# baudm/parseq

Measured on NVIDIA H100. Metric: images/sec PARSeq-S 32x128 AR+1refine, higher is better.
Workload: dtype bf16

## Files before the change

### include/parseq_b200.h

```cpp
#ifndef PARSEQ_B200_H_
#define PARSEQ_B200_H_

#include <stdint.h>

#ifdef __cplusplus
extern "C" {
#endif

typedef struct parseq_engine parseq_engine;
typedef void* parseq_stream_t;

typedef enum parseq_status {
  PARSEQ_OK = 0,
  PARSEQ_ERR_INVALID_ARG = -1,
  PARSEQ_ERR_UNSUPPORTED = -2,
  PARSEQ_ERR_CUDA = -3,
  PARSEQ_ERR_STATE = -4,
  PARSEQ_ERR_NO_DEVICE = -5
} parseq_status;

typedef struct parseq_config {
  int32_t img_h, img_w;
  int32_t patch_h, patch_w;
  int32_t embed_dim;
  int32_t enc_num_heads, enc_mlp_ratio, enc_depth;
  int32_t dec_num_heads, dec_mlp_ratio, dec_depth;
  int32_t max_label_length;
  int32_t num_tokens;
  int32_t max_batch;
  int32_t device;
  int32_t arch;
} parseq_config;

int parseq_create(const parseq_config* cfg, parseq_engine** out);
void parseq_destroy(parseq_engine* e);

int parseq_set_weight(parseq_engine* e, const char* key, const float* data, int64_t numel);
int parseq_num_weights(const parseq_engine* e);
const char* parseq_weight_key(const parseq_engine* e, int i, int64_t* numel);

int parseq_finalize(parseq_engine* e, parseq_stream_t stream);

typedef struct parseq_forward_args {
  int32_t batch;
  int32_t max_length;
  int32_t decode_ar;
  int32_t refine_iters;
  const int32_t* forced_ids;
  const int32_t* forced_refine;
  const uint32_t* class_mask;
  float* attn_maps;
} parseq_forward_args;

int parseq_forward(parseq_engine* e, const parseq_forward_args* args, const float* images,
                   float* logits, int32_t* ids, int32_t* steps, parseq_stream_t stream);

int parseq_forward_host(parseq_engine* e, const parseq_forward_args* args, const float* images_host,
                        float* logits_host, int32_t* ids_host, int32_t* steps_host,
                        parseq_stream_t stream);

int parseq_forward_u8(parseq_engine* e, const parseq_forward_args* args, const uint8_t* images_hwc,
                      float* logits, int32_t* ids, int32_t* steps, parseq_stream_t stream);
int parseq_forward_host_u8(parseq_engine* e, const parseq_forward_args* args, const uint8_t* images_hwc_host,
                           float* logits_host, int32_t* ids_host, int32_t* steps_host, parseq_stream_t stream);
typedef struct parseq_crops {
  const uint8_t* data;
  int64_t data_bytes;
  const int64_t* offsets;
  const int32_t* sizes;
  int32_t rotation;
  const int32_t* rotations;
} parseq_crops;
int parseq_resize_crops(parseq_engine* e, int32_t batch, const parseq_crops* crops, uint8_t* out_hwc, parseq_stream_t stream);
int parseq_forward_crops(parseq_engine* e, const parseq_forward_args* args, const parseq_crops* crops, float* logits,
                         int32_t* ids, int32_t* steps, parseq_stream_t stream);
int parseq_forward_host_crops(parseq_engine* e, const parseq_forward_args* args, const parseq_crops* crops,
                              float* logits_host, int32_t* ids_host, int32_t* steps_host, parseq_stream_t stream);
typedef struct parseq_orient_args {
  int32_t num_orientations;
  int32_t orientations[4];
  float min_confidence;
  int32_t* rotation_out;
  float* confidence_out;
} parseq_orient_args;
int parseq_forward_crops_oriented(parseq_engine* e, const parseq_forward_args* args, const parseq_crops* crops,
                                  const parseq_orient_args* orient, float* logits, int32_t* ids, int32_t* steps,
                                  parseq_stream_t stream);
typedef struct parseq_score_args {
  int32_t batch;
  int32_t num_candidates;
  const int32_t* per_image;
  const int32_t* targets;
  const int32_t* lengths;
  float* attn_maps;
} parseq_score_args;
int parseq_score(parseq_engine* e, const parseq_score_args* a, const float* images, float* scores, float* token_logprobs,
                 parseq_stream_t stream);
int parseq_score_u8(parseq_engine* e, const parseq_score_args* a, const uint8_t* images_hwc, float* scores,
                    float* token_logprobs, parseq_stream_t stream);
int parseq_score_check(const parseq_config* cfg, const parseq_score_args* a);

typedef struct parseq_beam_args {
  int32_t batch, beam_width, max_length;
  const uint32_t* class_mask;
  float* attn_maps;
} parseq_beam_args;
int parseq_beam_search(parseq_engine* e, const parseq_beam_args* a, const float* images, int32_t* ids, int32_t* lengths,
                       float* scores, parseq_stream_t stream);
int parseq_beam_search_u8(parseq_engine* e, const parseq_beam_args* a, const uint8_t* images_hwc, int32_t* ids,
                          int32_t* lengths, float* scores, parseq_stream_t stream);

typedef struct parseq_lexicon parseq_lexicon;
typedef struct parseq_lexicon_desc {
  int32_t num_nodes, num_edges;
  const int32_t* first_edge;
  const int32_t* edge_class;
  const int32_t* edge_child;
  const uint8_t* terminal;
} parseq_lexicon_desc;
int parseq_lexicon_check(const parseq_config* cfg, const parseq_lexicon_desc* d);
int parseq_lexicon_create(parseq_engine* e, const parseq_lexicon_desc* d, parseq_lexicon** out, parseq_stream_t stream);
void parseq_lexicon_destroy(parseq_lexicon* lx);
int parseq_beam_search_lexicon(parseq_engine* e, const parseq_beam_args* a, const parseq_lexicon* lx, const int32_t* roots,
                               const float* images, int32_t* ids, int32_t* lengths, float* scores, parseq_stream_t stream);
int parseq_beam_search_lexicon_u8(parseq_engine* e, const parseq_beam_args* a, const parseq_lexicon* lx,
                                  const int32_t* roots, const uint8_t* images_hwc, int32_t* ids, int32_t* lengths,
                                  float* scores, parseq_stream_t stream);

int parseq_postprocess(const float* logits, int32_t batch, int32_t num_steps, int32_t num_classes, int32_t eos_id,
                       int32_t* ids, int32_t* lengths, float* confidence, parseq_stream_t stream);

int parseq_encode(parseq_engine* e, int32_t batch, const float* images, float* memory,
                  parseq_stream_t stream);

int parseq_decode(parseq_engine* e, int32_t batch, int32_t ctx_len, int32_t num_queries, const int32_t* tgt,
                  const float* memory, const float* query, const uint8_t* query_mask, const uint8_t* padding_mask,
                  float* out, parseq_stream_t stream);
int parseq_decode_ex(parseq_engine* e, int32_t batch, int32_t ctx_len, int32_t num_queries, const int32_t* tgt,
                     const float* memory, const float* query, const uint8_t* query_mask, const uint8_t* padding_mask,
                     const uint8_t* content_mask, float* out, parseq_stream_t stream);
int parseq_head(parseq_engine* e, int32_t rows, const float* x, float* logits, parseq_stream_t stream);
int parseq_text_embed(parseq_engine* e, int32_t n, const int32_t* ids, float* out, parseq_stream_t stream);

int64_t parseq_kernel_launches(const parseq_engine* e);
int parseq_bench_tma_stream(void* buf, int64_t bytes, int cluster, int ctas, int nboxes, int nslot, int mode, void* sink,
                            parseq_stream_t stream);
int64_t parseq_debug_int(parseq_engine* e, const char* name);
int parseq_set_option(parseq_engine* e, const char* name, int64_t value);
int parseq_get_timing(parseq_engine* e, int category, double* ms, double* flops, int64_t* count);
int parseq_get_ar_profile(parseq_engine* e, uint64_t* out512);
const char* parseq_last_error(void);
const char* parseq_version(void);

int parseq_gemm_bf16(const void* A, int64_t lda, const void* W, int64_t ldw, const float* bias,
                     int M, int N, int K, int mode, float alpha, const float* resid, int64_t ldr,
                     int resid_mod, void* out, int64_t ldo, parseq_stream_t stream);
int parseq_gemm_ln_bf16(const void* A, int64_t lda, const void* W, int64_t ldw, const float* bias,
                        int M, int D, int K, float* x_inout, const float* gamma, const float* beta,
                        float eps, void* xn_bf16, parseq_stream_t stream);
int parseq_mlp_ln_bf16(const void* xn, const void* W1, const float* b1, const void* W2, const float* b2,
                       int M, int D, float* x_inout, const float* gamma, const float* beta, float eps,
                       void* xn_out_bf16, parseq_stream_t stream);
int parseq_layernorm_bf16(const float* x, const float* gamma, const float* beta, float eps, int M,
                          int D, void* y_bf16, float* y_f32_or_null, parseq_stream_t stream);
int parseq_enc_attention(const void* qkv_bf16, int B, int T, int D, int heads, void* out_bf16,
                         parseq_stream_t stream);
int parseq_qkv_attention_bf16(const void* xn_bf16, const void* W_qkv, const float* b_qkv, int B, int T, int D,
                              int heads, void* out_bf16, parseq_stream_t stream);
int parseq_head_lse_bf16(const void* A, int64_t lda, const void* W, int64_t ldw, const float* bias, int M, int N, int K,
                         const int32_t* tgt, float* part, float* tlogit, parseq_stream_t stream);
int parseq_head_topk_bf16(const void* A, int64_t lda, const void* W, int64_t ldw, const float* bias, int M, int N, int K,
                          int k, const uint32_t* mask, int mask_div, float* part, uint64_t* keys, parseq_stream_t stream);
typedef struct parseq_beam_select_args {
  const float* logits;
  const float* part;
  const uint64_t* keys;
  int32_t ntiles;
  int64_t row0, img_stride, slot_stride;
  int32_t batch, num_classes, beam_width, step, num_steps;
  const uint32_t* class_mask;
  int32_t mask_ld;
  const int32_t* ids_in;
  const float* score_in;
  const int32_t* len_in;
  const int32_t* st_in;
  int32_t* ids_out;
  float* score_out;
  int32_t* len_out;
  int32_t* st_out;
  int32_t* parent;
  int32_t ids_ld;
  int32_t* out_ids;
  int32_t* out_len;
  float* out_score;
  const int32_t* first_edge;
  const int32_t* edge_class;
  const int32_t* edge_child;
  const uint8_t* terminal;
  const int32_t* roots;
  const int32_t* node_in;
  int32_t* node_out;
} parseq_beam_select_args;
int parseq_beam_select(const parseq_beam_select_args* a, parseq_stream_t stream);

#ifdef __cplusplus
}
#endif
#endif
```

### parseq_b200/csrc/engine.cu

```cuda
#include <cuda.h>
#include <cuda_runtime.h>

#include <algorithm>
#include <cmath>
#include <cstdio>
#include <cstdlib>
#include <cstring>
#include <functional>
#include <map>
#include <mutex>
#include <set>
#include <string>
#include <type_traits>
#include <vector>

#include "../../include/parseq_b200.h"
#include "gemm.cuh"
#include "kernels.cuh"
#include "dec_ar.cuh"
#include "dec_ar2.cuh"
#include "gemm_ln.cuh"
#include "mlp_ln.cuh"
#include "attn_wgmma.cuh"
#include "qkv_attn.cuh"
#include "crops.cuh"
#include "orient.cuh"
#include "owners.h"

namespace {

constexpr int kMaxHeadClasses = 16384;
constexpr int kMaxLabelLength = 63;

thread_local std::string g_last_error;

int fail(int code, const std::string& msg) {
  g_last_error = msg;
  return code;
}
#define PQ_CUDA(expr)                                                                              \
  do {                                                                                             \
    cudaError_t _e = (expr);                                                                       \
    if (_e != cudaSuccess)                                                                         \
      return fail(PARSEQ_ERR_CUDA, std::string(#expr) + " -> " + cudaGetErrorString(_e));          \
  } while (0)
#define PQ_TRY(expr)                 \
  do {                               \
    int _r = (expr);                 \
    if (_r != PARSEQ_OK) return _r;  \
  } while (0)

typedef CUresult (*PFN_encodeTiled)(CUtensorMap*, CUtensorMapDataType, cuuint32_t, void*, const cuuint64_t*,
                                    const cuuint64_t*, const cuuint32_t*, const cuuint32_t*, CUtensorMapInterleave,
                                    CUtensorMapSwizzle, CUtensorMapL2promotion, CUtensorMapFloatOOBfill);
PFN_encodeTiled g_encode = nullptr;

int load_driver_api() {
  if (g_encode != nullptr) return PARSEQ_OK;
  void* fn = nullptr;
  cudaDriverEntryPointQueryResult qres;
  cudaError_t e = cudaGetDriverEntryPoint("cuTensorMapEncodeTiled", &fn, cudaEnableDefault, &qres);
  if (e != cudaSuccess || fn == nullptr || qres != cudaDriverEntryPointSuccess)
    return fail(PARSEQ_ERR_CUDA, "cuTensorMapEncodeTiled not available from the driver");
  g_encode = reinterpret_cast<PFN_encodeTiled>(fn);
  return PARSEQ_OK;
}

int make_tmap(CUtensorMap* tm, const void* ptr, int esize, long long rows, long long cols, long long ld, int box_cols,
              int box_rows) {
  PQ_TRY(load_driver_api());
  if ((reinterpret_cast<uintptr_t>(ptr) & 15u) != 0 || ((ld * esize) & 15) != 0)
    return fail(PARSEQ_ERR_INVALID_ARG, "GEMM operand must be 16-byte aligned with a 16-byte multiple row stride");
  cuuint64_t dims[2] = {static_cast<cuuint64_t>(cols), static_cast<cuuint64_t>(rows)};
  cuuint64_t strides[1] = {static_cast<cuuint64_t>(ld) * static_cast<cuuint64_t>(esize)};
  cuuint32_t box[2] = {static_cast<cuuint32_t>(box_cols), static_cast<cuuint32_t>(box_rows)};
  cuuint32_t estr[2] = {1, 1};
  CUresult r = g_encode(tm, esize == 2 ? CU_TENSOR_MAP_DATA_TYPE_BFLOAT16 : CU_TENSOR_MAP_DATA_TYPE_FLOAT32, 2,
                        const_cast<void*>(ptr), dims, strides, box, estr,
                        CU_TENSOR_MAP_INTERLEAVE_NONE, CU_TENSOR_MAP_SWIZZLE_128B, CU_TENSOR_MAP_L2_PROMOTION_L2_256B,
                        CU_TENSOR_MAP_FLOAT_OOB_FILL_NONE);
  if (r != CUDA_SUCCESS) return fail(PARSEQ_ERR_CUDA, "cuTensorMapEncodeTiled failed: " + std::to_string(int(r)));
  return PARSEQ_OK;
}

int make_tmap3d(CUtensorMap* tm, const void* ptr, long long d0, long long d1, long long d2, long long ld1, long long ld2,
                int box_d0, int box_d1) {
  PQ_TRY(load_driver_api());
  if ((reinterpret_cast<uintptr_t>(ptr) & 15u) != 0 || ((ld1 * 2) & 15) != 0 || ((ld2 * 2) & 15) != 0)
    return fail(PARSEQ_ERR_INVALID_ARG, "tensor map operand must be 16-byte aligned with 16-byte multiple strides");
  cuuint64_t dims[3] = {static_cast<cuuint64_t>(d0), static_cast<cuuint64_t>(d1), static_cast<cuuint64_t>(d2)};
  cuuint64_t strides[2] = {static_cast<cuuint64_t>(ld1) * 2u, static_cast<cuuint64_t>(ld2) * 2u};
  cuuint32_t box[3] = {static_cast<cuuint32_t>(box_d0), static_cast<cuuint32_t>(box_d1), 1u};
  cuuint32_t estr[3] = {1, 1, 1};
  CUresult r = g_encode(tm, CU_TENSOR_MAP_DATA_TYPE_BFLOAT16, 3, const_cast<void*>(ptr), dims, strides, box, estr,
                        CU_TENSOR_MAP_INTERLEAVE_NONE, CU_TENSOR_MAP_SWIZZLE_128B, CU_TENSOR_MAP_L2_PROMOTION_L2_256B,
                        CU_TENSOR_MAP_FLOAT_OOB_FILL_NONE);
  if (r != CUDA_SUCCESS) return fail(PARSEQ_ERR_CUDA, "cuTensorMapEncodeTiled(3d) failed: " + std::to_string(int(r)));
  return PARSEQ_OK;
}

int make_tmap_kv4d(CUtensorMap* tm, const void* ptr, int T, int max_batch, int panels, int box_t) {
  PQ_TRY(load_driver_api());
  if ((reinterpret_cast<uintptr_t>(ptr) & 15u) != 0)
    return fail(PARSEQ_ERR_INVALID_ARG, "tensor map operand must be 16-byte aligned");
  const cuuint64_t row = 128;
  cuuint64_t dims[4] = {64, static_cast<cuuint64_t>(T), static_cast<cuuint64_t>(max_batch), static_cast<cuuint64_t>(panels)};
  cuuint64_t strides[3] = {row, row * T, row * T * max_batch};
  cuuint32_t box[4] = {64, static_cast<cuuint32_t>(box_t), 1u, 1u};
  cuuint32_t estr[4] = {1, 1, 1, 1};
  CUresult r = g_encode(tm, CU_TENSOR_MAP_DATA_TYPE_BFLOAT16, 4, const_cast<void*>(ptr), dims, strides, box, estr,
                        CU_TENSOR_MAP_INTERLEAVE_NONE, CU_TENSOR_MAP_SWIZZLE_128B, CU_TENSOR_MAP_L2_PROMOTION_L2_256B,
                        CU_TENSOR_MAP_FLOAT_OOB_FILL_NONE);
  if (r != CUDA_SUCCESS) return fail(PARSEQ_ERR_CUDA, "cuTensorMapEncodeTiled(K/V 4d) failed: " + std::to_string(int(r)));
  return PARSEQ_OK;
}

uint16_t f32_to_bf16_rne(float f) {
  uint32_t u;
  std::memcpy(&u, &f, 4);
  if ((u & 0x7fffffffu) > 0x7f800000u) return static_cast<uint16_t>((u >> 16) | 0x40u);
  u += 0x7fffu + ((u >> 16) & 1u);
  return static_cast<uint16_t>(u >> 16);
}

struct LaunchOpts {
  int sm_count = 0;
  bool use_pdl = true;
  int ln_cta_group = 0;
  int ln_split = 0;
  int mlp_cta_group = 0;
  bool pair_pdl = false;
  int gemm_stages = 0;
  int attn_impl = 0;
  int ln_clusters = 0;
};
LaunchOpts g_default_opts;

int ensure_sm_count(LaunchOpts& o) {
  if (o.sm_count == 0) {
    int dev = 0;
    PQ_CUDA(cudaGetDevice(&dev));
    PQ_CUDA(cudaDeviceGetAttribute(&o.sm_count, cudaDevAttrMultiProcessorCount, dev));
  }
  return PARSEQ_OK;
}

struct LaunchConfig {
  cudaLaunchConfig_t cfg{};
  cudaLaunchAttribute attr[2];
  LaunchConfig(dim3 grid, dim3 block, size_t smem, cudaStream_t st, unsigned cluster, bool pdl) {
    cfg.gridDim = grid;
    cfg.blockDim = block;
    cfg.dynamicSmemBytes = smem;
    cfg.stream = st;
    cfg.attrs = attr;
    if (cluster > 0) {
      attr[cfg.numAttrs].id = cudaLaunchAttributeClusterDimension;
      attr[cfg.numAttrs].val.clusterDim.x = cluster;
      attr[cfg.numAttrs].val.clusterDim.y = 1;
      attr[cfg.numAttrs].val.clusterDim.z = 1;
      ++cfg.numAttrs;
    }
    if (pdl) {
      attr[cfg.numAttrs].id = cudaLaunchAttributeProgrammaticStreamSerialization;
      attr[cfg.numAttrs].val.programmaticStreamSerializationAllowed = 1;
      ++cfg.numAttrs;
    }
  }
  LaunchConfig(const LaunchConfig&) = delete;
  LaunchConfig& operator=(const LaunchConfig&) = delete;
};

template <typename... KArgs, typename... Args>
int launch_ex(const LaunchConfig& lc, void (*kern)(KArgs...), const Args&... args) {
  PQ_CUDA(cudaLaunchKernelEx(&lc.cfg, kern, static_cast<KArgs>(args)...));
  return PARSEQ_OK;
}
template <typename... KArgs, typename... Args>
int launch_k(const LaunchOpts& lo, void (*kern)(KArgs...), dim3 grid, dim3 block, size_t smem, cudaStream_t st, const Args&... args) {
  return launch_ex(LaunchConfig(grid, block, smem, st, 0, lo.use_pdl), kern, args...);
}
bool cluster_pdl(const LaunchOpts& lo, int cg) { return lo.use_pdl && (cg == 1 || lo.pair_pdl); }

template <typename F>
int dispatch_width(int D, const char* what, F&& f) {
  switch (D) {
    case 192: return f(std::integral_constant<int, 192>{});
    case 384: return f(std::integral_constant<int, 384>{});
    case 768: return f(std::integral_constant<int, 768>{});
    default: return fail(PARSEQ_ERR_UNSUPPORTED, std::string(what) + ": embed_dim must be 192, 384 or 768");
  }
}

template <int EPI, int STORE>
int launch_gemm_cfg(const LaunchOpts& lo, const CUtensorMap& ta, const CUtensorMap& tb, const CUtensorMap& to,
                    const pq::GemmParams& p, int tiles, cudaStream_t st) {
  const int grid = tiles < lo.sm_count ? tiles : lo.sm_count;
  return launch_k(lo, pq::gemm_bf16_wgmma_kernel<EPI, STORE>, dim3(static_cast<unsigned>(grid)), dim3(pq::GEMM_THREADS),
                  pq::GemmCfg::smem_bytes<STORE != pq::ST_REG>(), st, ta, tb, to, p);
}

size_t head_smem_bytes(int C, int D) {
  return ((static_cast<size_t>(C) * (D / 2 + 1) * 4 + 15) / 16) * 16 + static_cast<size_t>(pq::HEAD_ROWS) * D * 4 +
         4 * pq::HEAD_ROWS * 128 * 4 + pq::HEAD_ROWS * 128 * 4;
}
int ln_head_argmax_launch(const LaunchOpts& lo, const float* y, const float* g, const float* b, float eps, const __nv_bfloat16* Wh, const float* bh,
                          int M, int C, int D, float* logits, long long logits_ld, int* ids, int ids_ld, int nq, int dst_off,
                          const int* forced, int forced_ld, const uint32_t* mask, cudaStream_t st) {
  if (C > 128) return fail(PARSEQ_ERR_UNSUPPORTED, "head kernel covers at most 128 classes");
  const dim3 grid((M + pq::HEAD_ROWS - 1) / pq::HEAD_ROWS), block(384);
  const size_t sm = head_smem_bytes(C, D);
  switch (D) {
    case 192: return launch_k(lo, pq::dec_ln_head_argmax_kernel<192>, grid, block, sm, st, y, g, b, eps, Wh, bh, M, C, logits,
                              logits_ld, ids, ids_ld, nq, dst_off, forced, forced_ld, mask);
    case 384: return launch_k(lo, pq::dec_ln_head_argmax_kernel<384>, grid, block, sm, st, y, g, b, eps, Wh, bh, M, C, logits,
                              logits_ld, ids, ids_ld, nq, dst_off, forced, forced_ld, mask);
    case 768: return launch_k(lo, pq::dec_ln_head_argmax_kernel<768>, grid, block, sm, st, y, g, b, eps, Wh, bh, M, C, logits,
                              logits_ld, ids, ids_ld, nq, dst_off, forced, forced_ld, mask);
    default: return fail(PARSEQ_ERR_UNSUPPORTED, "head kernel: embed_dim must be 192, 384 or 768");
  }
}

template <int D, int MT, int CS, bool HS, bool WIDE, int IDP>
constexpr auto ar2_kernel() {
  if constexpr (IDP == 64) {
    if constexpr (WIDE) return pq::dec_ar2_long_wide_kernel<D, MT, CS, HS>;
    else return pq::dec_ar2_long_kernel<D, MT, CS, HS>;
  } else {
    if constexpr (WIDE) return pq::dec_ar2_wide_kernel<D, MT, CS, HS>;
    else return pq::dec_ar2_kernel<D, MT, CS, HS>;
  }
}
template <typename... KArgs>
int set_smem(void (*kern)(KArgs...), size_t bytes) {
  PQ_CUDA(cudaFuncSetAttribute(kern, cudaFuncAttributeMaxDynamicSharedMemorySize, static_cast<int>(bytes)));
  return PARSEQ_OK;
}
template <int D, int MT, int CS, bool WIDE, int IDP>
int ar2_attr() {
  PQ_TRY(set_smem(ar2_kernel<D, MT, CS, false, WIDE, IDP>(), pq::dec_ar2_smem_bytes<D, MT, CS, IDP>()));
  if constexpr (MT == 1 && CS == 8 && D / 64 <= CS)
    PQ_TRY(set_smem(ar2_kernel<D, MT, CS, true, WIDE, IDP>(), pq::dec_ar2_smem_bytes<D, MT, CS, IDP>()));
  return PARSEQ_OK;
}
template <bool WIDE, int IDP>
int ar2_set_attributes() {
  PQ_TRY((ar2_attr<192, 1, 8, WIDE, IDP>())); PQ_TRY((ar2_attr<192, 2, 8, WIDE, IDP>())); PQ_TRY((ar2_attr<384, 1, 8, WIDE, IDP>()));
  PQ_TRY((ar2_attr<384, 2, 8, WIDE, IDP>())); PQ_TRY((ar2_attr<768, 1, 8, WIDE, IDP>()));
  PQ_TRY((ar2_attr<192, 1, 6, WIDE, IDP>())); PQ_TRY((ar2_attr<192, 2, 6, WIDE, IDP>())); PQ_TRY((ar2_attr<384, 1, 6, WIDE, IDP>()));
  PQ_TRY((ar2_attr<384, 2, 6, WIDE, IDP>())); PQ_TRY((ar2_attr<768, 1, 6, WIDE, IDP>()));
  return PARSEQ_OK;
}

template <int D, int MODE>
int gemm_ln_attr() { return set_smem(pq::gemm_ln_fused_kernel<D, MODE>, pq::GemmLnCfg<D, MODE>::kSmemBytes); }
template <int D, int CG>
int mlp_ln_attr() { return set_smem(pq::mlp_ln_fused_kernel<D, CG>, pq::MlpLnCfg<D, CG>::kSmemBytes); }
template <int NK>
int attn_wgmma_attr() { return set_smem(pq::enc_attention_wgmma_kernel<NK>, pq::atw_smem_bytes<NK>()); }
template <int D>
int qkv_attn_attr() { return set_smem(pq::enc_qkv_attn_kernel<D>, pq::QkvAttnCfg::kSmemBytes); }
template <int EPI, int STORE>
int gemm_attr() { return set_smem(pq::gemm_bf16_wgmma_kernel<EPI, STORE>, pq::GemmCfg::smem_bytes<STORE != pq::ST_REG>()); }
constexpr int kTmaBenchSmem = 12 * pq::A2_SLOT + 1024 + 256;

int init_kernel_attributes() {
  PQ_TRY(set_smem(pq::dec_ar_kernel<192, 1>, pq::dec_ar_smem_bytes<192>()));
  PQ_TRY(set_smem(pq::dec_ar_kernel<192, 2>, pq::dec_ar_smem_bytes<192>()));
  PQ_TRY(set_smem(pq::dec_ar_kernel<384, 1>, pq::dec_ar_smem_bytes<384>()));
  PQ_TRY(set_smem(pq::dec_ar_kernel<384, 2>, pq::dec_ar_smem_bytes<384>()));
  PQ_TRY(set_smem(pq::dec_ar_kernel<768, 1>, pq::dec_ar_smem_bytes<768>()));
  PQ_TRY(set_smem(pq::dec_ar_kernel<768, 2>, pq::dec_ar_smem_bytes<768>()));
  PQ_TRY((ar2_set_attributes<false, 32>()));
  PQ_TRY((ar2_set_attributes<true, 32>()));
  PQ_TRY((ar2_set_attributes<false, 64>()));
  PQ_TRY((ar2_set_attributes<true, 64>()));
  PQ_TRY(set_smem(pq::dec_ln_head_argmax_kernel<192>, 120 * 1024));
  PQ_TRY(set_smem(pq::dec_ln_head_argmax_kernel<384>, 160 * 1024));
  PQ_TRY(set_smem(pq::dec_ln_head_argmax_kernel<768>, 226 * 1024));
  PQ_TRY((gemm_ln_attr<192, 0>())); PQ_TRY((gemm_ln_attr<384, 0>())); PQ_TRY((gemm_ln_attr<192, 1>()));
  PQ_TRY((gemm_ln_attr<384, 1>())); PQ_TRY((gemm_ln_attr<384, 2>()));
  PQ_TRY((mlp_ln_attr<192, 1>())); PQ_TRY((mlp_ln_attr<384, 1>())); PQ_TRY((mlp_ln_attr<192, 2>())); PQ_TRY((mlp_ln_attr<384, 2>()));
  PQ_TRY((attn_wgmma_attr<128>())); PQ_TRY((attn_wgmma_attr<256>()));
  PQ_TRY((qkv_attn_attr<192>())); PQ_TRY((qkv_attn_attr<384>()));
  PQ_TRY((gemm_attr<pq::EPI_F32, pq::ST_REG>()));
  PQ_TRY((gemm_attr<pq::EPI_F32_RESID, pq::ST_REG>()));
  PQ_TRY((gemm_attr<pq::EPI_BF16, pq::ST_REG>()));
  PQ_TRY((gemm_attr<pq::EPI_BF16, pq::ST_TMA_2D>()));
  PQ_TRY((gemm_attr<pq::EPI_BF16, pq::ST_TMA_3D>()));
  PQ_TRY((gemm_attr<pq::EPI_GELU_BF16, pq::ST_REG>()));
  PQ_TRY((gemm_attr<pq::EPI_GELU_BF16, pq::ST_TMA_2D>()));
  PQ_TRY(set_smem(pq::gemm_bf16_lse_kernel, pq::GemmCfg::smem_bytes<false>()));
  PQ_TRY(set_smem(pq::gemm_bf16_topk_kernel, pq::GemmCfg::smem_bytes<false>()));
  PQ_TRY(set_smem(pq::tma_stream_bench_kernel, kTmaBenchSmem));
  int dev = 0, optin = 0;
  PQ_CUDA(cudaGetDevice(&dev));
  PQ_CUDA(cudaDeviceGetAttribute(&optin, cudaDevAttrMaxSharedMemoryPerBlockOptin, dev));
  PQ_TRY(set_smem(pq::crop_resize_bicubic_kernel, static_cast<size_t>(optin)));
  return PARSEQ_OK;
}

int ensure_kernel_attributes() {
  static std::mutex mu;
  static std::set<int> done;
  int dev = 0;
  PQ_CUDA(cudaGetDevice(&dev));
  std::lock_guard<std::mutex> lock(mu);
  if (done.count(dev) != 0) return PARSEQ_OK;
  PQ_TRY(init_kernel_attributes());
  done.insert(dev);
  return PARSEQ_OK;
}

int gemm_launch(LaunchOpts& lo, const void* A, long long lda, const void* W, long long ldw, const float* bias, int M, int N,
                int K, int mode, float alpha, const float* resid, long long ldr, int resid_mod, void* out, long long ldo,
                cudaStream_t st, long long blocked_rows = 0) {
  if (M <= 0 || N <= 0 || K <= 0) return fail(PARSEQ_ERR_INVALID_ARG, "gemm: empty problem");
  if (mode != pq::EPI_F32 && mode != pq::EPI_BF16 && mode != pq::EPI_GELU_BF16)
    return fail(PARSEQ_ERR_INVALID_ARG, "gemm: mode must be 0 (fp32), 1 (bf16) or 2 (GELU bf16)");
  PQ_TRY(ensure_sm_count(lo));
  CUtensorMap ta, tb, to;
  PQ_TRY(make_tmap(&ta, A, 2, M, K, lda, pq::GEMM_BLOCK_K, pq::GEMM_BLOCK_M));
  PQ_TRY(make_tmap(&tb, W, 2, N, K, ldw, pq::GEMM_BLOCK_K, pq::GEMM_BLOCK_N));
  pq::GemmParams p;
  p.M = M; p.N = N; p.K = K; p.alpha = alpha; p.bias = bias;
  p.resid = resid; p.ldr = ldr; p.resid_mod = resid_mod; p.out = out; p.ldo = ldo;
  const int esz = (mode == pq::EPI_F32) ? 4 : 2;
  bool vec = ((reinterpret_cast<uintptr_t>(out) & 7u) == 0) && ((ldo * esz) % 8 == 0);
  if (resid != nullptr) vec = vec && ((reinterpret_cast<uintptr_t>(resid) & 7u) == 0) && ((ldr * 4) % 8 == 0);
  p.vec_ok = vec ? 1 : 0;
  int store = pq::ST_REG;
  if (blocked_rows > 0) {
    if (mode != pq::EPI_BF16 || N % 64 != 0 || blocked_rows < M || (reinterpret_cast<uintptr_t>(out) & 15u) != 0)
      return fail(PARSEQ_ERR_INVALID_ARG, "gemm: blocked output needs a bf16 epilogue, N % 64 == 0 and rows >= M");
    PQ_TRY(make_tmap3d(&to, out, 64, M, N / 64, 64, 64 * blocked_rows, 64, pq::GEMM_BLOCK_M));
    store = pq::ST_TMA_3D;
  } else if (mode != pq::EPI_F32 && (reinterpret_cast<uintptr_t>(out) & 15u) == 0 && (ldo * 2) % 16 == 0 && ldo >= N) {
    PQ_TRY(make_tmap(&to, out, 2, M, N, ldo, 64, pq::GEMM_BLOCK_M));
    store = pq::ST_TMA_2D;
  } else {
    to = ta;
  }
  p.max_stages = lo.gemm_stages;
  p.num_m_tiles = (M + pq::GEMM_BLOCK_M - 1) / pq::GEMM_BLOCK_M;
  p.num_n_tiles = (N + pq::GEMM_BLOCK_N - 1) / pq::GEMM_BLOCK_N;
  const int tiles = p.num_m_tiles * p.num_n_tiles;
  if (mode == pq::EPI_F32)
    return resid != nullptr ? launch_gemm_cfg<pq::EPI_F32_RESID, pq::ST_REG>(lo, ta, tb, to, p, tiles, st)
                            : launch_gemm_cfg<pq::EPI_F32, pq::ST_REG>(lo, ta, tb, to, p, tiles, st);
  if (mode == pq::EPI_BF16) {
    if (store == pq::ST_TMA_3D) return launch_gemm_cfg<pq::EPI_BF16, pq::ST_TMA_3D>(lo, ta, tb, to, p, tiles, st);
    return store == pq::ST_TMA_2D ? launch_gemm_cfg<pq::EPI_BF16, pq::ST_TMA_2D>(lo, ta, tb, to, p, tiles, st)
                                  : launch_gemm_cfg<pq::EPI_BF16, pq::ST_REG>(lo, ta, tb, to, p, tiles, st);
  }
  return store == pq::ST_TMA_2D ? launch_gemm_cfg<pq::EPI_GELU_BF16, pq::ST_TMA_2D>(lo, ta, tb, to, p, tiles, st)
                                : launch_gemm_cfg<pq::EPI_GELU_BF16, pq::ST_REG>(lo, ta, tb, to, p, tiles, st);
}

int gemm_lse_launch(LaunchOpts& lo, const void* A, long long lda, const void* W, long long ldw, const float* bias, int M, int N,
                    int K, const int* tgt, float2* part, float* tlogit, cudaStream_t st) {
  if (M <= 0 || N <= 0 || K <= 0) return fail(PARSEQ_ERR_INVALID_ARG, "gemm: empty problem");
  PQ_TRY(ensure_sm_count(lo));
  CUtensorMap ta, tb;
  PQ_TRY(make_tmap(&ta, A, 2, M, K, lda, pq::GEMM_BLOCK_K, pq::GEMM_BLOCK_M));
  PQ_TRY(make_tmap(&tb, W, 2, N, K, ldw, pq::GEMM_BLOCK_K, pq::GEMM_BLOCK_N));
  pq::GemmParams p{};
  p.M = M; p.N = N; p.K = K; p.alpha = 1.0f; p.bias = bias;
  p.out = part;
  p.max_stages = lo.gemm_stages;
  p.num_m_tiles = (M + pq::GEMM_BLOCK_M - 1) / pq::GEMM_BLOCK_M;
  p.num_n_tiles = (N + pq::GEMM_BLOCK_N - 1) / pq::GEMM_BLOCK_N;
  p.lse_tgt = tgt;
  p.lse_tlogit = tlogit;
  const int tiles = p.num_m_tiles * p.num_n_tiles;
  return launch_k(lo, pq::gemm_bf16_lse_kernel, dim3(static_cast<unsigned>(tiles < lo.sm_count ? tiles : lo.sm_count)),
                  dim3(pq::GEMM_THREADS), pq::GemmCfg::smem_bytes<false>(), st, ta, tb, ta, p);
}

int gemm_topk_launch(LaunchOpts& lo, const void* A, long long lda, const void* W, long long ldw, const float* bias, int M, int N,
                     int K, int k, const uint32_t* mask, int mask_div, float2* part, unsigned long long* keys, cudaStream_t st) {
  if (M <= 0 || N <= 0 || K <= 0) return fail(PARSEQ_ERR_INVALID_ARG, "gemm: empty problem");
  PQ_TRY(ensure_sm_count(lo));
  CUtensorMap ta, tb;
  PQ_TRY(make_tmap(&ta, A, 2, M, K, lda, pq::GEMM_BLOCK_K, pq::GEMM_BLOCK_M));
  PQ_TRY(make_tmap(&tb, W, 2, N, K, ldw, pq::GEMM_BLOCK_K, pq::GEMM_BLOCK_N));
  pq::GemmParams p{};
  p.M = M; p.N = N; p.K = K; p.alpha = 1.0f; p.bias = bias;
  p.out = part;
  p.max_stages = lo.gemm_stages;
  p.num_m_tiles = (M + pq::GEMM_BLOCK_M - 1) / pq::GEMM_BLOCK_M;
  p.num_n_tiles = (N + pq::GEMM_BLOCK_N - 1) / pq::GEMM_BLOCK_N;
  p.topk_keys = keys;
  p.topk_k = k;
  p.topk_mask = mask;
  p.topk_mask_div = mask_div;
  const int tiles = p.num_m_tiles * p.num_n_tiles;
  return launch_k(lo, pq::gemm_bf16_topk_kernel, dim3(static_cast<unsigned>(tiles < lo.sm_count ? tiles : lo.sm_count)),
                  dim3(pq::GEMM_THREADS), pq::GemmCfg::smem_bytes<false>(), st, ta, tb, ta, p);
}

bool gemm_ln_supported(int D) { return D == 192 || D == 384; }
template <int D, int MODE>
int launch_gemm_ln(LaunchOpts& lo, const void* A, long long lda, const void* W, long long ldw, const float* bias, int M, int K, float* x,
                   const float* gamma, const float* beta, float eps, void* xn, cudaStream_t st) {
  using Cfg = pq::GemmLnCfg<D, MODE>;
  CUtensorMap ta, tb, tx;
  PQ_TRY(make_tmap(&ta, A, 2, M, K, lda, pq::GEMM_BLOCK_K, Cfg::kABox));
  PQ_TRY(make_tmap(&tb, W, 2, D, K, ldw, pq::GEMM_BLOCK_K, Cfg::kBox));
  if ((reinterpret_cast<uintptr_t>(x) & 7u) != 0 || (reinterpret_cast<uintptr_t>(xn) & 3u) != 0)
    return fail(PARSEQ_ERR_INVALID_ARG, "gemm_ln: x must be 8-byte and xn 4-byte aligned");
  pq::GemmLnParams p;
  p.M = M; p.K = K; p.bias = bias; p.gamma = gamma; p.beta = beta; p.eps = eps;
  p.num_m_tiles = (M + Cfg::kTileM - 1) / Cfg::kTileM;
  int clusters = p.num_m_tiles;
  if constexpr (MODE == 2) {
    PQ_TRY(make_tmap(&tx, x, 4, M, D, D, Cfg::kXBoxCols, pq::GLN_BLOCK_M));
    if (lo.ln_clusters == 0) {
      const LaunchConfig occ(dim3(static_cast<unsigned>(lo.sm_count / Cfg::kCG * Cfg::kCG)), dim3(pq::GLN_THREADS),
                             Cfg::kSmemBytes, st, Cfg::kCG, false);
      PQ_CUDA(cudaOccupancyMaxActiveClusters(&lo.ln_clusters, pq::gemm_ln_fused_kernel<D, MODE>, &occ.cfg));
      if (lo.ln_clusters <= 0) return fail(PARSEQ_ERR_CUDA, "gemm_ln: no cluster of the persistent kernel fits the device");
    }
    clusters = std::min(p.num_m_tiles, lo.ln_clusters);
  } else {
    tx = ta;
  }
  return launch_ex(LaunchConfig(dim3(static_cast<unsigned>(clusters * Cfg::kCG)), dim3(pq::GLN_THREADS), Cfg::kSmemBytes, st,
                                Cfg::kCG, cluster_pdl(lo, Cfg::kCG)),
                   pq::gemm_ln_fused_kernel<D, MODE>, ta, tb, tx, x, reinterpret_cast<__nv_bfloat16*>(xn), p);
}
int gemm_ln_launch(LaunchOpts& lo, const void* A, long long lda, const void* W, long long ldw, const float* bias, int M, int D,
                   int K, float* x, const float* gamma, const float* beta, float eps, void* xn, cudaStream_t st) {
  if (M <= 0 || K <= 0) return fail(PARSEQ_ERR_INVALID_ARG, "gemm_ln: empty problem");
  PQ_TRY(ensure_sm_count(lo));
  PQ_TRY(load_driver_api());
  if (D == 384 && lo.ln_split != 1)
    return launch_gemm_ln<384, 2>(lo, A, lda, W, ldw, bias, M, K, x, gamma, beta, eps, xn, st);
  if (lo.ln_cta_group == 2) {
    if (D == 384) return launch_gemm_ln<384, 1>(lo, A, lda, W, ldw, bias, M, K, x, gamma, beta, eps, xn, st);
    if (D == 192) return launch_gemm_ln<192, 1>(lo, A, lda, W, ldw, bias, M, K, x, gamma, beta, eps, xn, st);
  }
  if (D == 384) return launch_gemm_ln<384, 0>(lo, A, lda, W, ldw, bias, M, K, x, gamma, beta, eps, xn, st);
  if (D == 192) return launch_gemm_ln<192, 0>(lo, A, lda, W, ldw, bias, M, K, x, gamma, beta, eps, xn, st);
  return fail(PARSEQ_ERR_UNSUPPORTED, "gemm_ln: embed_dim must be 192 or 384");
}

template <int D, int CG>
int launch_mlp_ln(const LaunchOpts& lo, const void* xn, const void* W1, const float* b1, const void* W2, const float* b2, int M,
                  float* x, const float* gamma, const float* beta, float eps, void* xn_out, cudaStream_t st) {
  using Cfg = pq::MlpLnCfg<D, CG>;
  if ((reinterpret_cast<uintptr_t>(x) & 7u) != 0 || (reinterpret_cast<uintptr_t>(xn_out) & 3u) != 0)
    return fail(PARSEQ_ERR_INVALID_ARG, "mlp_ln: x must be 8-byte and xn_out 4-byte aligned");
  CUtensorMap txn, tw1, tw2;
  PQ_TRY(make_tmap(&txn, xn, 2, M, D, D, 64, pq::GLN_BLOCK_M));
  PQ_TRY(make_tmap(&tw1, W1, 2, Cfg::kH, D, D, 64, Cfg::kW1Rows));
  PQ_TRY(make_tmap(&tw2, W2, 2, D, Cfg::kH, Cfg::kH, 64, Cfg::kW2Rows));
  pq::MlpLnParams p;
  p.M = M; p.b1 = b1; p.b2 = b2; p.gamma = gamma; p.beta = beta; p.eps = eps;
  p.num_m_tiles = (M + pq::GLN_BLOCK_M * CG - 1) / (pq::GLN_BLOCK_M * CG);
  return launch_ex(LaunchConfig(dim3(static_cast<unsigned>(p.num_m_tiles * CG)), dim3(pq::MLP_THREADS), Cfg::kSmemBytes, st, CG,
                                cluster_pdl(lo, CG)),
                   pq::mlp_ln_fused_kernel<D, CG>, txn, tw1, tw2, x, reinterpret_cast<__nv_bfloat16*>(xn_out), p);
}
int mlp_ln_launch(LaunchOpts& lo, const void* xn, const void* W1, const float* b1, const void* W2, const float* b2, int M, int D,
                  float* x, const float* gamma, const float* beta, float eps, void* xn_out, cudaStream_t st) {
  if (M <= 0) return fail(PARSEQ_ERR_INVALID_ARG, "mlp_ln: empty problem");
  PQ_TRY(ensure_sm_count(lo));
  PQ_TRY(load_driver_api());
  const int CG = lo.mlp_cta_group ? lo.mlp_cta_group : 2;
  if (CG == 2) {
    if (D == 384) return launch_mlp_ln<384, 2>(lo, xn, W1, b1, W2, b2, M, x, gamma, beta, eps, xn_out, st);
    if (D == 192) return launch_mlp_ln<192, 2>(lo, xn, W1, b1, W2, b2, M, x, gamma, beta, eps, xn_out, st);
  }
  if (D == 384) return launch_mlp_ln<384, 1>(lo, xn, W1, b1, W2, b2, M, x, gamma, beta, eps, xn_out, st);
  if (D == 192) return launch_mlp_ln<192, 1>(lo, xn, W1, b1, W2, b2, M, x, gamma, beta, eps, xn_out, st);
  return fail(PARSEQ_ERR_UNSUPPORTED, "mlp_ln: embed_dim must be 192 or 384 (hidden width 4 * embed_dim)");
}

int layernorm_launch(const LaunchOpts& lo, const float* x, const float* g, const float* b, float eps, int M, int D, void* y, float* y32,
                     cudaStream_t st, const float* add = nullptr, int add_mod = 1, float* xw = nullptr) {
  const int rows_per_block = 8;
  const int grid = (M + rows_per_block - 1) / rows_per_block;
  __nv_bfloat16* yb = reinterpret_cast<__nv_bfloat16*>(y);
  switch (D) {
    case 192: return launch_k(lo, pq::layernorm_kernel<192>, dim3(grid), dim3(256), 0, st, x, g, b, eps, M, yb, y32, add, add_mod, xw);
    case 384: return launch_k(lo, pq::layernorm_kernel<384>, dim3(grid), dim3(256), 0, st, x, g, b, eps, M, yb, y32, add, add_mod, xw);
    case 768: return launch_k(lo, pq::layernorm_kernel<768>, dim3(grid), dim3(256), 0, st, x, g, b, eps, M, yb, y32, add, add_mod, xw);
    default: return fail(PARSEQ_ERR_UNSUPPORTED, "layernorm: embed_dim must be 192, 384 or 768");
  }
}

int enc_attention_launch(const LaunchOpts& lo, const void* qkv, int B, int T, int D, int heads, void* out, cudaStream_t st) {
  if (D != heads * pq::ATT_DH) return fail(PARSEQ_ERR_UNSUPPORTED, "encoder attention kernels cover head_dim=64");
  if (lo.attn_impl == 1 && T <= 256) {
    const dim3 grid(static_cast<unsigned>(B * heads), static_cast<unsigned>((T + 127) / 128));
    const __nv_bfloat16* q = reinterpret_cast<const __nv_bfloat16*>(qkv);
    __nv_bfloat16* o = reinterpret_cast<__nv_bfloat16*>(out);
    if (T <= 128)
      return launch_k(lo, pq::enc_attention_wgmma_kernel<128>, grid, dim3(pq::ATW_THREADS), pq::atw_smem_bytes<128>(), st, q, o, T, D, heads);
    return launch_k(lo, pq::enc_attention_wgmma_kernel<256>, grid, dim3(pq::ATW_THREADS), pq::atw_smem_bytes<256>(), st, q, o, T, D, heads);
  }
  if (T != pq::ATT_T) {
    return launch_k(lo, pq::enc_attention_any_kernel, dim3(B * heads, (T + pq::ATT_T - 1) / pq::ATT_T), dim3(256), 0, st,
                    reinterpret_cast<const __nv_bfloat16*>(qkv), reinterpret_cast<__nv_bfloat16*>(out), T, D, heads);
  }
  return launch_k(lo, pq::enc_attention_kernel, dim3(B * heads), dim3(256), 0, st,
                  reinterpret_cast<const __nv_bfloat16*>(qkv), reinterpret_cast<__nv_bfloat16*>(out), D, heads);
}

bool qkv_attn_supported(int T, int D, int heads) { return T == pq::ATT_T && D == heads * pq::ATT_DH && (D == 192 || D == 384); }
int qkv_attn_launch(LaunchOpts& lo, const void* xn, const void* W, const float* bias, int B, int T, int D, int heads, void* out,
                    cudaStream_t st) {
  if (B <= 0) return fail(PARSEQ_ERR_INVALID_ARG, "qkv_attn: empty batch");
  if (!qkv_attn_supported(T, D, heads))
    return fail(PARSEQ_ERR_UNSUPPORTED, "qkv_attn: T = 128, head_dim 64 and embed_dim 192 or 384 only");
  if ((reinterpret_cast<uintptr_t>(out) & 15u) != 0) return fail(PARSEQ_ERR_INVALID_ARG, "qkv_attn: out must be 16-byte aligned");
  PQ_TRY(ensure_sm_count(lo));
  CUtensorMap tx, tw;
  PQ_TRY(make_tmap(&tx, xn, 2, static_cast<long long>(B) * T, D, D, pq::GEMM_BLOCK_K, pq::ATT_T));
  PQ_TRY(make_tmap(&tw, W, 2, 3 * D, D, D, pq::GEMM_BLOCK_K, pq::ATT_DH));
  const int items = B * heads;
  const dim3 grid(static_cast<unsigned>(items < lo.sm_count ? items : lo.sm_count));
  __nv_bfloat16* o = reinterpret_cast<__nv_bfloat16*>(out);
  if (D == 192)
    return launch_k(lo, pq::enc_qkv_attn_kernel<192>, grid, dim3(pq::QA_THREADS), pq::QkvAttnCfg::kSmemBytes, st, tx, tw, bias, o, items);
  return launch_k(lo, pq::enc_qkv_attn_kernel<384>, grid, dim3(pq::QA_THREADS), pq::QkvAttnCfg::kSmemBytes, st, tx, tw, bias, o, items);
}

int make_stream(Stream* s) {
  cudaStream_t h = nullptr;
  PQ_CUDA(cudaStreamCreateWithFlags(&h, cudaStreamNonBlocking));
  *s = Stream(h);
  return PARSEQ_OK;
}
int make_event(Event* ev) {
  cudaEvent_t h = nullptr;
  PQ_CUDA(cudaEventCreateWithFlags(&h, cudaEventDisableTiming));
  *ev = Event(h);
  return PARSEQ_OK;
}

struct Slot {
  std::string key;
  std::string pub;
  long long numel;
  bool bf16;
  DevBuf<unsigned char> dev;
  bool set;
};

struct Workspace {
  DevBuf<__nv_bfloat16> a_pe, xn, qkv, att, hid;
  DevBuf<float> x;
  DevBuf<float> vt_rows;
  DevBuf<__nv_bfloat16> mem, ckv;
  std::vector<DevBuf<__nv_bfloat16>> ckv_deep;
  DevBuf<__nv_bfloat16> ar_sa, ar_ca, ar_hd;
  DevBuf<float> ar_y, ar_qc, ar_part;
  DevBuf<int> ar_ids;
  DevBuf<unsigned int> ar_bar;
  DevBuf<unsigned long long> ar_prof;
  Event ev_enc;
  struct Stage {
    DevBuf<__nv_bfloat16> sa, yn, ca, hd;
    DevBuf<float> y, qc;
    DevBuf<int> ids_ar, ids_ctx;
    DevBuf<float> cx;
    std::vector<DevBuf<__nv_bfloat16>> kvc;
    DevBuf<float2> lse_part;
    DevBuf<float> lse_tlogit;
    struct Beam {
      int rows = 0;
      DevBuf<int> ids[2];
      DevBuf<float> score[2];
      DevBuf<int> len[2];
      DevBuf<int> st[2];
      DevBuf<int> parent;
      DevBuf<float> logits;
      DevBuf<float2> part;
      DevBuf<unsigned long long> keys;
      std::vector<DevBuf<__nv_bfloat16>> kvc;
      DevBuf<int> node[2];
    } bm;
    Stream stream;
    Event ev_done;
  };
  std::vector<Stage> stages;
  DevBuf<float> in_images, out_logits;
  DevBuf<int> out_ids, out_steps;
  DevBuf<float> out_maps;
  DevBuf<uint8_t> in_images_u8;
  DevBuf<uint32_t> in_mask;
  DevBuf<pq::CropDesc> crop_tab;
  DevBuf<int> sc_meta;
  DevBuf<unsigned char> sc_causal;
  DevBuf<float2> sc_vt_part;
  long long beam_bytes = 0;
  DevBuf<int> lex_roots;
  DevBuf<int> or_rd, or_steps;
  DevBuf<float> or_conf;
};

}

struct parseq_engine : Workspace {
  parseq_config cfg;
  int D, T, Kp, Me, Md, L, V, C, gh, gw, dh_dec;
  int ids_ld = 32;
  int arch = 0, Tp = 0;
  std::map<std::string, int> pub_index;
  int chunk;
  std::vector<Slot> slots;
  std::map<std::string, int> index;
  bool finalized = false;
  bool broken = false;
  LaunchOpts lo;
  long long launches = 0;
  bool timing = false;
  struct TimedLaunch { int cat; double flops; Event a, b; };
  std::vector<TimedLaunch> timed;
  std::vector<Event> event_pool;
  int cur_cat = 5;
  DevBuf<__nv_bfloat16> kvtab;
  DevBuf<float> qs;
  int dec_chunk = 128;
  int ar_kernel = 2;
  pq::DecAr2Maps ar2_maps[2];
  bool ar2_maps_ok = false;
  int ar2_clusters[3][2] = {{0, 0}, {0, 0}, {0, 0}};
  int ar2_occ[3][2] = {{0, 0}, {0, 0}, {0, 0}};
  int ar_last_cs = 0;
  int ar_last_per = 0, ar_last_ncl = 0;
  int ar_last_mt = 0, ar_last_hs = 0, ar_last_wide = 0, ar_last_idp = 0;
  int ar_last_path = -1;
  int ar_cs = 0;
  int ar_clusters_override = 0;
  int fuse_mlp = 0;
  int fuse_ln = 3;
  bool ar_prof_on = false;
  int max_batch = 512;
  Stream main;
  Stream copy;
  Event ev_c[3];
  Event ev_in, ev_out;
  int mask_ld = 0;
  std::vector<pq::CropDesc> crop_descs;
  long long crop_base = 0;
  DevBuf<uint8_t> crop_stage;
  bool use_graph = true;
  long long orient_rereads = 0, orient_readings = 0;
  struct GraphEntry { GraphExec exec; long long kernels; };
  std::map<std::vector<int>, GraphEntry> graphs;

  void* w(const std::string& k) const { return slots[index.at(k)].dev; }
  const float* wf(const std::string& k) const { return reinterpret_cast<const float*>(w(k)); }
  const __nv_bfloat16* wb(const std::string& k) const { return reinterpret_cast<const __nv_bfloat16*>(w(k)); }
};

struct parseq_lexicon {
  int device = 0, C = 0, V = 0, E = 0;
  DevBuf<int> first_edge;
  DevBuf<int> edge_class;
  DevBuf<int> edge_child;
  DevBuf<unsigned char> terminal;
};

template <typename T>
int DevBuf<T>::alloc(long long n) {
  reset();
  void* p = nullptr;
  PQ_CUDA(cudaMalloc(&p, static_cast<size_t>(n) * sizeof(T)));
  p_ = static_cast<T*>(p);
  n_ = n;
  g_live_bytes += bytes();
  return PARSEQ_OK;
}

template <typename T>
int DevBuf<T>::grow(const parseq_engine* e, long long n) {
  if (n <= n_) return PARSEQ_OK;
  if (p_ != nullptr) {
    PQ_CUDA(cudaStreamSynchronize(e->main));
    PQ_CUDA(cudaStreamSynchronize(e->copy));
  }
  return alloc(n);
}

namespace {

void add_slot(parseq_engine* e, const std::string& key, long long numel, bool bf16) {
  std::string pub = key;
  if (e->arch == 1 && key.rfind("encoder.", 0) == 0) pub = key.substr(8);
  e->index[key] = static_cast<int>(e->slots.size());
  e->pub_index[pub] = static_cast<int>(e->slots.size());
  e->slots.push_back(Slot{key, pub, numel, bf16, {}, false});
}

int check_ready(const parseq_engine* e, bool weights = true) {
  if (e == nullptr) return fail(PARSEQ_ERR_INVALID_ARG, "null argument");
  if (e->broken) return fail(PARSEQ_ERR_STATE, "engine workspace is gone (a failed resize): destroy the handle");
  if (weights && !e->finalized)
    return fail(PARSEQ_ERR_STATE, "parseq_finalize has not been called after the last weight update");
  return PARSEQ_OK;
}

int enter_main(parseq_engine* e, cudaStream_t user) {
  PQ_CUDA(cudaEventRecord(e->ev_in, user));
  PQ_CUDA(cudaStreamWaitEvent(e->main, e->ev_in, 0));
  return PARSEQ_OK;
}
int leave_main(parseq_engine* e, cudaStream_t user) {
  PQ_CUDA(cudaEventRecord(e->ev_out, e->main));
  PQ_CUDA(cudaStreamWaitEvent(user, e->ev_out, 0));
  return PARSEQ_OK;
}

long long image_bytes(const parseq_engine* e, bool u8) { return 3ll * e->cfg.img_h * e->cfg.img_w * (u8 ? 1 : 4); }

int alloc_workspace(parseq_engine* e) {
  const long long R = static_cast<long long>(e->chunk) * e->T;
  const long long RB = static_cast<long long>(e->max_batch) * e->T;
  const long long Rd = static_cast<long long>(e->dec_chunk) * e->L;
  const int D = e->D;
  PQ_TRY(e->a_pe.alloc(R * e->Kp));
  PQ_TRY(e->x.alloc(R * D));
  PQ_TRY(e->xn.alloc(R * D));
  PQ_TRY(e->qkv.alloc(R * 3 * D));
  PQ_TRY(e->att.alloc(R * D));
  PQ_TRY(e->hid.alloc(R * e->Me));
  PQ_TRY(e->mem.alloc(RB * D));
  PQ_TRY(e->ckv.alloc(RB * 2 * D));
  if (e->cfg.dec_depth > 1) {
    e->ckv_deep.resize(static_cast<size_t>(e->cfg.dec_depth - 1));
    for (auto& c : e->ckv_deep) PQ_TRY(c.alloc(RB * 2 * D));
  }
  PQ_TRY(e->ar_sa.alloc(1ll * e->max_batch * D));
  PQ_TRY(e->ar_ca.alloc(1ll * e->max_batch * D));
  PQ_TRY(e->ar_hd.alloc(1ll * e->max_batch * e->Md));
  PQ_TRY(e->ar_y.alloc(1ll * e->max_batch * D));
  PQ_TRY(e->ar_qc.alloc(1ll * e->max_batch * D));
// ... 2002 lines not shown
  return beam_lexicon_call(e, a, lx, roots, images, false, ids, lengths, scores, stream);
}

int parseq_beam_search_lexicon_u8(parseq_engine* e, const parseq_beam_args* a, const parseq_lexicon* lx,
                                  const int32_t* roots, const uint8_t* images_hwc, int32_t* ids, int32_t* lengths,
                                  float* scores, parseq_stream_t stream) {
  return beam_lexicon_call(e, a, lx, roots, images_hwc, true, ids, lengths, scores, stream);
}

int parseq_postprocess(const float* logits, int32_t batch, int32_t num_steps, int32_t num_classes, int32_t eos_id, int32_t* ids,
                       int32_t* lengths, float* confidence, parseq_stream_t stream) {
  if (logits == nullptr || ids == nullptr || lengths == nullptr || confidence == nullptr)
    return fail(PARSEQ_ERR_INVALID_ARG, "null argument");
  if (batch <= 0) return batch == 0 ? PARSEQ_OK : fail(PARSEQ_ERR_INVALID_ARG, "negative batch");
  pq::postprocess_kernel<<<(batch + 7) / 8, 256, 0, reinterpret_cast<cudaStream_t>(stream)>>>(logits, batch, num_steps, num_classes,
                                                                                              eos_id, ids, lengths, confidence);
  PQ_CUDA(cudaGetLastError());
  return PARSEQ_OK;
}

int parseq_encode(parseq_engine* e, int32_t batch, const float* images, float* memory, parseq_stream_t stream) {
  if (images == nullptr || memory == nullptr) return fail(PARSEQ_ERR_INVALID_ARG, "null argument");
  PQ_TRY(check_ready(e));
  PQ_CUDA(cudaSetDevice(e->cfg.device));
  cudaStream_t user = reinterpret_cast<cudaStream_t>(stream);
  PQ_TRY(enter_main(e, user));
  const long long img_sz = 3ll * e->cfg.img_h * e->cfg.img_w;
  for (int b0 = 0; b0 < batch; b0 += e->chunk) {
    const int B = (batch - b0 < e->chunk) ? (batch - b0) : e->chunk;
    PQ_TRY(encode_chunk(e, images + b0 * img_sz, false, B, e->mem, memory + 1ll * b0 * e->T * e->D, e->main));
  }
  return leave_main(e, user);
}

int parseq_decode(parseq_engine* e, int32_t batch, int32_t ctx_len, int32_t num_queries, const int32_t* tgt, const float* memory,
                  const float* query, const uint8_t* query_mask, const uint8_t* padding_mask, float* out,
                  parseq_stream_t stream) {
  return parseq_decode_ex(e, batch, ctx_len, num_queries, tgt, memory, query, query_mask, padding_mask, nullptr, out, stream);
}

int parseq_decode_ex(parseq_engine* e, int32_t batch, int32_t ctx_len, int32_t num_queries, const int32_t* tgt,
                     const float* memory, const float* query, const uint8_t* query_mask, const uint8_t* padding_mask,
                     const uint8_t* content_mask, float* out, parseq_stream_t stream) {
  if (tgt == nullptr || memory == nullptr || out == nullptr) return fail(PARSEQ_ERR_INVALID_ARG, "null argument");
  PQ_TRY(check_ready(e));
  if (e->arch != 0) return fail(PARSEQ_ERR_UNSUPPORTED, "decode: PARSeq only");
  if (batch < 0 || ctx_len < 1 || ctx_len > e->L || num_queries < 1 || num_queries > e->L)
    return fail(PARSEQ_ERR_INVALID_ARG, "decode: 1 <= context length, queries <= max_label_length + 1");
  if (batch == 0) return PARSEQ_OK;
  PQ_CUDA(cudaSetDevice(e->cfg.device));
  cudaStream_t user = reinterpret_cast<cudaStream_t>(stream);
  PQ_TRY(enter_main(e, user));
  const int D = e->D, T = e->T, J = ctx_len, NQ = num_queries;
  parseq_engine::Stage& sg = e->stages[0];
  cudaStream_t st = e->main;
  for (int b0 = 0; b0 < batch; b0 += e->dec_chunk) {
    const int Bc = (batch - b0 < e->dec_chunk) ? (batch - b0) : e->dec_chunk;
    const long long n4 = 1ll * Bc * T * D / 4;
    pq::f32_to_bf16_kernel<<<static_cast<unsigned>(std::min<long long>((n4 + 255) / 256, 132ll * 8)), 256, 0, st>>>(
        reinterpret_cast<const float4*>(memory + 1ll * b0 * T * D), reinterpret_cast<uint2*>(e->mem.get()), n4);
    PQ_CUDA(cudaGetLastError());
    PQ_TRY(cross_kv(e, Bc));
    pq::copy_ids_kernel<<<(Bc * e->ids_ld + 255) / 256, 256, 0, st>>>(tgt + 1ll * b0 * J, J, sg.ids_ctx, Bc, e->ids_ld);
    PQ_CUDA(cudaGetLastError());
    e->launches += 2;
    DecodeExtras ex;
    ex.query = query ? query + 1ll * b0 * NQ * D : nullptr;
    ex.qmask = query_mask;
    ex.pmask = padding_mask ? padding_mask + 1ll * b0 * J : nullptr;
    ex.cmask = content_mask;
    ex.out_norm = out + 1ll * b0 * NQ * D;
    PQ_TRY(decode_pass(e, sg, 0, Bc, NQ, 0, J, 0, sg.ids_ctx, nullptr, 0, nullptr, 0, nullptr, 0, nullptr, st, &ex));
  }
  return leave_main(e, user);
}

int parseq_head(parseq_engine* e, int32_t rows, const float* x, float* logits, parseq_stream_t stream) {
  if (x == nullptr || logits == nullptr) return fail(PARSEQ_ERR_INVALID_ARG, "null argument");
  PQ_TRY(check_ready(e));
  if (rows <= 0) return rows == 0 ? PARSEQ_OK : fail(PARSEQ_ERR_INVALID_ARG, "negative rows");
  PQ_CUDA(cudaSetDevice(e->cfg.device));
  cudaStream_t user = reinterpret_cast<cudaStream_t>(stream);
  PQ_TRY(enter_main(e, user));
  const int D = e->D;
  const int cap = e->dec_chunk * e->L;
  parseq_engine::Stage& sg = e->stages[0];
  for (int r0 = 0; r0 < rows; r0 += cap) {
    const int n = (rows - r0 < cap) ? (rows - r0) : cap;
    const long long n4 = 1ll * n * D / 4;
    pq::f32_to_bf16_kernel<<<static_cast<unsigned>(std::min<long long>((n4 + 255) / 256, 132ll * 8)), 256, 0, e->main>>>(
        reinterpret_cast<const float4*>(x + 1ll * r0 * D), reinterpret_cast<uint2*>(sg.yn.get()), n4);
    PQ_CUDA(cudaGetLastError());
    e->launches++;
    e->cur_cat = CAT_DEC_GEMM;
    PQ_TRY(gemm(e, sg.yn, D, e->w("head.weight"), D, e->wf("head.bias"), n, e->C, D, pq::EPI_F32, 1.0f, nullptr, 0, 0,
                logits + 1ll * r0 * e->C, e->C, e->main));
  }
  return leave_main(e, user);
}

int parseq_text_embed(parseq_engine* e, int32_t n, const int32_t* ids, float* out, parseq_stream_t stream) {
  if (e == nullptr || ids == nullptr || out == nullptr) return fail(PARSEQ_ERR_INVALID_ARG, "null argument");
  if (e->arch != 0) return fail(PARSEQ_ERR_UNSUPPORTED, "text_embed: PARSeq only");
  if (n <= 0) return n == 0 ? PARSEQ_OK : fail(PARSEQ_ERR_INVALID_ARG, "negative count");
  if (!e->slots[e->index.at("text_embed.embedding.weight")].set) return fail(PARSEQ_ERR_STATE, "weights not set");
  PQ_CUDA(cudaSetDevice(e->cfg.device));
  const long long total = 1ll * n * e->D;
  pq::text_embed_kernel<<<static_cast<unsigned>(std::min<long long>((total + 255) / 256, 132ll * 8)), 256, 0,
                          reinterpret_cast<cudaStream_t>(stream)>>>(ids, e->wf("text_embed.embedding.weight"), out, n, e->D, e->V,
                                                                    std::sqrt(static_cast<float>(e->D)));
  PQ_CUDA(cudaGetLastError());
  return PARSEQ_OK;
}

int parseq_bench_tma_stream(void* buf, int64_t bytes, int cluster, int ctas, int nboxes, int nslot, int mode, void* sink,
                            parseq_stream_t stream) {
  if (buf == nullptr || sink == nullptr || cluster < 1 || cluster > 8 || ctas % cluster != 0 || nslot < 1 || nslot > 12)
    return fail(PARSEQ_ERR_INVALID_ARG, "bench_tma_stream: bad arguments");
  const long long rows_total = 8192;
  const int blocks = static_cast<int>(bytes / (rows_total * 128));
  if (blocks < 1) return fail(PARSEQ_ERR_INVALID_ARG, "bench_tma_stream: buffer too small");
  PQ_TRY(ensure_kernel_attributes());
  CUtensorMap map;
  PQ_TRY(make_tmap3d(&map, buf, 64, rows_total, blocks, 64, 64 * rows_total, 64, 128));
  return launch_ex(LaunchConfig(dim3(static_cast<unsigned>(ctas)), dim3(pq::A2_THREADS + 32), kTmaBenchSmem,
                                reinterpret_cast<cudaStream_t>(stream), cluster > 1 ? static_cast<unsigned>(cluster) : 0, false),
                   pq::tma_stream_bench_kernel, map, nboxes, nslot, static_cast<int>(rows_total / 128), blocks, mode,
                   static_cast<unsigned int*>(sink));
}

int64_t parseq_debug_int(parseq_engine* e, const char* name) {
  if (name == nullptr) return -1;
  const std::string n(name);
  if (n == "ln_clusters") return (e ? e->lo : g_default_opts).ln_clusters;
  if (n == "live_device_bytes") return g_live_bytes;
  if (n == "live_cuda_objects") return g_live_objects;
  if (e == nullptr) return -1;
  if (n == "ar2_occupancy_mt1_cs8") return e->ar2_occ[1][0];
  if (n == "ar2_occupancy_mt2_cs8") return e->ar2_occ[2][0];
  if (n == "ar2_occupancy_mt1_cs6") return e->ar2_occ[1][1];
  if (n == "ar2_occupancy_mt2_cs6") return e->ar2_occ[2][1];
  if (n == "ar_last_cluster_size") return e->ar_last_cs;
  if (n == "ar_last_per") return e->ar_last_per;
  if (n == "ar_last_clusters") return e->ar_last_ncl;
  if (n == "ar_last_mt") return e->ar_last_mt;
  if (n == "ar_last_head_split") return e->ar_last_hs;
  if (n == "ar_last_wide") return e->ar_last_wide;
  if (n == "ar_last_ids_pitch") return e->ar_last_idp;
  if (n == "ar_last_path") return e->ar_last_path;
  if (n == "sm_count") return e->lo.sm_count;
  if (n == "beam_bytes") return e->beam_bytes;
  if (n == "orient_rereads") return e->orient_rereads;
  if (n == "orient_readings") return e->orient_readings;
  return -1;
}
int64_t parseq_kernel_launches(const parseq_engine* e) { return e ? e->launches : 0; }

int parseq_set_option(parseq_engine* e, const char* name, int64_t value) {
  if (name == nullptr) return fail(PARSEQ_ERR_INVALID_ARG, "null option");
  const std::string n(name);
  LaunchOpts& lo = e ? e->lo : g_default_opts;
  if (n == "block_n") {
    if (value != 0 && value != 64 && value != 128 && value != 192 && value != 256)
      return fail(PARSEQ_ERR_INVALID_ARG, "block_n: 0/64/128/192/256");
    return PARSEQ_OK;
  }
  if (n == "cta_group") {
    if (value < 0 || value > 2) return fail(PARSEQ_ERR_INVALID_ARG, "cta_group: 0 (auto) / 1 / 2");
    return PARSEQ_OK;
  }
  if (n == "attn_impl") { lo.attn_impl = value != 0 ? 1 : 0; if (e) e->graphs.clear(); return PARSEQ_OK; }
  if (n == "pdl") { lo.use_pdl = value != 0; if (e) e->graphs.clear(); return PARSEQ_OK; }
  if (n == "gemm_stages") {
    if (value < 0 || value == 1) return fail(PARSEQ_ERR_INVALID_ARG, "gemm_stages: 0 (full ring) or >= 2");
    lo.gemm_stages = static_cast<int>(value);
    if (e) e->graphs.clear();
    return PARSEQ_OK;
  }
  if (n == "ln_cta_group") {
    if (value < 0 || value > 2) return fail(PARSEQ_ERR_INVALID_ARG, "ln_cta_group: 0 (auto) / 1 / 2");
    lo.ln_cta_group = static_cast<int>(value);
    if (e) e->graphs.clear();
    return PARSEQ_OK;
  }
  if (n == "ln_split") {
    if (value < 0 || value > 2) return fail(PARSEQ_ERR_INVALID_ARG, "ln_split: 0 (auto) / 1 (off) / 2 (on)");
    lo.ln_split = static_cast<int>(value);
    if (e) e->graphs.clear();
    return PARSEQ_OK;
  }
  if (n == "mlp_cta_group") {
    if (value < 0 || value > 2) return fail(PARSEQ_ERR_INVALID_ARG, "mlp_cta_group: 0 (auto) / 1 / 2");
    lo.mlp_cta_group = static_cast<int>(value);
    if (e) e->graphs.clear();
    return PARSEQ_OK;
  }
  if (n == "pair_pdl") { lo.pair_pdl = value != 0; if (e) e->graphs.clear(); return PARSEQ_OK; }
  if (n == "fuse_mlp") {
    if (e == nullptr) return fail(PARSEQ_ERR_INVALID_ARG, "null engine");
    e->fuse_mlp = value != 0 ? 1 : 0;
    e->graphs.clear();
    return PARSEQ_OK;
  }
  if (n == "fuse_ln") {
    if (e == nullptr) return fail(PARSEQ_ERR_INVALID_ARG, "null engine");
    e->fuse_ln = static_cast<int>(value) & 7;
    e->graphs.clear();
    return PARSEQ_OK;
  }
  if (e == nullptr) return fail(PARSEQ_ERR_INVALID_ARG, "null engine");
  if (n == "timing") {
    e->timing = value != 0;
    for (auto& t : e->timed) { e->event_pool.push_back(std::move(t.a)); e->event_pool.push_back(std::move(t.b)); }
    e->timed.clear();
    return PARSEQ_OK;
  }
  if (n == "use_graph") { e->use_graph = value != 0; return PARSEQ_OK; }
  if (n == "ar_prof") { e->ar_prof_on = value != 0; e->graphs.clear(); return PARSEQ_OK; }
  if (n == "ar_clusters") {
    if (value < 0 || value > 1024) return fail(PARSEQ_ERR_INVALID_ARG, "ar_clusters out of range");
    e->ar_clusters_override = static_cast<int>(value);
    for (auto& r : e->ar2_clusters) r[0] = r[1] = 0;
    e->graphs.clear();
    return PARSEQ_OK;
  }
  if (n == "ar_cluster_size") {
    if (value != 0 && value != 6 && value != 8) return fail(PARSEQ_ERR_INVALID_ARG, "ar_cluster_size: 0 (auto) / 6 / 8");
    e->ar_cs = static_cast<int>(value);
    e->graphs.clear();
    return PARSEQ_OK;
  }
  if (n == "ar_kernel") {
    if (value < 0 || value > 2) return fail(PARSEQ_ERR_INVALID_ARG, "ar_kernel: 0 / 1 / 2");
    if (value == 1)
      if (const char* why = grid_barrier_limit(e)) return fail(PARSEQ_ERR_UNSUPPORTED, why);
    e->ar_kernel = static_cast<int>(value);
    e->graphs.clear();
    return PARSEQ_OK;
  }
  if (n == "chunk" || n == "max_batch" || n == "dec_chunk") {
    if (value <= 0 || value > 8192) return fail(PARSEQ_ERR_INVALID_ARG, "chunk / max_batch / dec_chunk out of range");
    int chunk = e->chunk, dec_chunk = e->dec_chunk, max_batch = e->max_batch;
    if (n == "chunk") chunk = static_cast<int>(value);
    else if (n == "dec_chunk") dec_chunk = static_cast<int>(value);
    else { max_batch = static_cast<int>(value); chunk = max_batch; }
    if (chunk > max_batch) chunk = max_batch;
    if (dec_chunk > max_batch) dec_chunk = max_batch;
    if ((max_batch + dec_chunk - 1) / dec_chunk > 64) return fail(PARSEQ_ERR_INVALID_ARG, "too many decoder chains");
    PQ_CUDA(cudaSetDevice(e->cfg.device));
    PQ_CUDA(cudaDeviceSynchronize());
    const int old_chunk = e->chunk, old_dec = e->dec_chunk, old_max = e->max_batch;
    free_workspace(e);
    e->chunk = chunk; e->dec_chunk = dec_chunk; e->max_batch = max_batch;
    int r = alloc_workspace(e);
    if (r != PARSEQ_OK) {
      const std::string why = g_last_error;
      free_workspace(e);
      e->chunk = old_chunk; e->dec_chunk = old_dec; e->max_batch = old_max;
      if (alloc_workspace(e) != PARSEQ_OK) { e->finalized = false; free_workspace(e); e->broken = true; }
      return fail(r, why);
    }
    return PARSEQ_OK;
  }
  return fail(PARSEQ_ERR_INVALID_ARG, "unknown option: " + n);
}

int parseq_get_ar_profile(parseq_engine* e, uint64_t* out512) {
  if (e == nullptr || out512 == nullptr) return fail(PARSEQ_ERR_INVALID_ARG, "null argument");
  PQ_CUDA(cudaMemcpy(out512, e->ar_prof, 32 * 16 * 8, cudaMemcpyDeviceToHost));
  return PARSEQ_OK;
}

int parseq_get_timing(parseq_engine* e, int category, double* ms, double* flops, int64_t* count) {
  if (e == nullptr || category < 0 || category >= CAT_COUNT) return fail(PARSEQ_ERR_INVALID_ARG, "bad timing query");
  double tms = 0.0, tf = 0.0;
  int64_t n = 0;
  for (auto& t : e->timed) {
    if (t.cat != category) continue;
    float dt = 0.f;
    cudaError_t ce = cudaEventElapsedTime(&dt, t.a, t.b);
    if (ce != cudaSuccess) return fail(PARSEQ_ERR_CUDA, std::string("timing readback: ") + cudaGetErrorString(ce));
    tms += dt; tf += t.flops; ++n;
  }
  if (ms) *ms = tms;
  if (flops) *flops = tf;
  if (count) *count = n;
  return PARSEQ_OK;
}

int parseq_gemm_bf16(const void* A, int64_t lda, const void* W, int64_t ldw, const float* bias, int M, int N, int K,
                     int mode, float alpha, const float* resid, int64_t ldr, int resid_mod, void* out, int64_t ldo,
                     parseq_stream_t stream) {
  if (mode < 0 || mode > 2) return fail(PARSEQ_ERR_INVALID_ARG, "bad epilogue mode");
  PQ_TRY(ensure_kernel_attributes());
  return gemm_launch(g_default_opts, A, lda, W, ldw, bias, M, N, K, mode, alpha, resid, ldr, resid_mod, out, ldo,
                     reinterpret_cast<cudaStream_t>(stream));
}
int parseq_gemm_ln_bf16(const void* A, int64_t lda, const void* W, int64_t ldw, const float* bias, int M, int D, int K,
                         float* x_inout, const float* gamma, const float* beta, float eps, void* xn_bf16,
                         parseq_stream_t stream) {
  PQ_TRY(ensure_kernel_attributes());
  return gemm_ln_launch(g_default_opts, A, lda, W, ldw, bias, M, D, K, x_inout, gamma, beta, eps, xn_bf16, reinterpret_cast<cudaStream_t>(stream));
}
int parseq_mlp_ln_bf16(const void* xn, const void* W1, const float* b1, const void* W2, const float* b2, int M, int D,
                       float* x_inout, const float* gamma, const float* beta, float eps, void* xn_out_bf16, parseq_stream_t stream) {
  PQ_TRY(ensure_kernel_attributes());
  return mlp_ln_launch(g_default_opts, xn, W1, b1, W2, b2, M, D, x_inout, gamma, beta, eps, xn_out_bf16,
                       reinterpret_cast<cudaStream_t>(stream));
}
int parseq_layernorm_bf16(const float* x, const float* gamma, const float* beta, float eps, int M, int D, void* y_bf16,
                          float* y_f32_or_null, parseq_stream_t stream) {
  PQ_TRY(ensure_kernel_attributes());
  return layernorm_launch(g_default_opts, x, gamma, beta, eps, M, D, y_bf16, y_f32_or_null, reinterpret_cast<cudaStream_t>(stream));
}
int parseq_enc_attention(const void* qkv_bf16, int B, int T, int D, int heads, void* out_bf16, parseq_stream_t stream) {
  PQ_TRY(ensure_kernel_attributes());
  PQ_TRY(ensure_sm_count(g_default_opts));
  return enc_attention_launch(g_default_opts, qkv_bf16, B, T, D, heads, out_bf16, reinterpret_cast<cudaStream_t>(stream));
}
int parseq_qkv_attention_bf16(const void* xn_bf16, const void* W_qkv, const float* b_qkv, int B, int T, int D, int heads,
                              void* out_bf16, parseq_stream_t stream) {
  PQ_TRY(ensure_kernel_attributes());
  return qkv_attn_launch(g_default_opts, xn_bf16, W_qkv, b_qkv, B, T, D, heads, out_bf16, reinterpret_cast<cudaStream_t>(stream));
}
int parseq_head_lse_bf16(const void* A, int64_t lda, const void* W, int64_t ldw, const float* bias, int M, int N, int K,
                         const int32_t* tgt, float* part, float* tlogit, parseq_stream_t stream) {
  if (part == nullptr || (tgt == nullptr) != (tlogit == nullptr))
    return fail(PARSEQ_ERR_INVALID_ARG, "head_lse: part is required, tgt and tlogit go together");
  PQ_TRY(ensure_kernel_attributes());
  return gemm_lse_launch(g_default_opts, A, lda, W, ldw, bias, M, N, K, tgt, reinterpret_cast<float2*>(part), tlogit,
                         reinterpret_cast<cudaStream_t>(stream));
}
int parseq_head_topk_bf16(const void* A, int64_t lda, const void* W, int64_t ldw, const float* bias, int M, int N, int K,
                          int k, const uint32_t* mask, int mask_div, float* part, uint64_t* keys, parseq_stream_t stream) {
  if (k < 1 || k > pq::BEAM_TOPK_LD) return fail(PARSEQ_ERR_INVALID_ARG, "head_topk: k must be in 1..16");
  if (part == nullptr || keys == nullptr) return fail(PARSEQ_ERR_INVALID_ARG, "head_topk: part and keys are required");
  if (mask != nullptr && mask_div < 1) return fail(PARSEQ_ERR_INVALID_ARG, "head_topk: mask_div must be >= 1");
  PQ_TRY(ensure_kernel_attributes());
  return gemm_topk_launch(g_default_opts, A, lda, W, ldw, bias, M, N, K, k, mask, mask != nullptr ? mask_div : 1,
                          reinterpret_cast<float2*>(part), reinterpret_cast<unsigned long long*>(keys),
                          reinterpret_cast<cudaStream_t>(stream));
}
int parseq_beam_select(const parseq_beam_select_args* a, parseq_stream_t stream) {
  if (a == nullptr) return fail(PARSEQ_ERR_INVALID_ARG, "beam_select: null arguments");
  const int C = a->num_classes, K = a->beam_width;
  const bool lex = a->first_edge != nullptr;
  if (a->batch < 1 || C < 1) return fail(PARSEQ_ERR_INVALID_ARG, "beam_select: batch and num_classes must be >= 1");
  if (K < 1 || K > pq::BEAM_MAX) return fail(PARSEQ_ERR_INVALID_ARG, "beam_select: beam_width must be in 1..16");
  if (a->ntiles != (C + pq::GEMM_BLOCK_N - 1) / pq::GEMM_BLOCK_N)
    return fail(PARSEQ_ERR_INVALID_ARG, "beam_select: ntiles must be ceil(num_classes / 128)");
  if (a->step < 0 || a->step >= a->num_steps) return fail(PARSEQ_ERR_INVALID_ARG, "beam_select: need 0 <= step < num_steps");
  if (a->ids_ld <= a->num_steps) return fail(PARSEQ_ERR_INVALID_ARG, "beam_select: ids_ld must exceed num_steps");
  if (a->logits == nullptr && (a->keys == nullptr || lex))
    return fail(PARSEQ_ERR_INVALID_ARG, "beam_select: logits are required without keys and with a lexicon");
  if (a->keys != nullptr && a->part == nullptr) return fail(PARSEQ_ERR_INVALID_ARG, "beam_select: keys need part");
  if (a->class_mask != nullptr && a->mask_ld < (C + 31) / 32)
    return fail(PARSEQ_ERR_INVALID_ARG, "beam_select: mask_ld must be >= ceil(num_classes / 32)");
  if (a->ids_in == nullptr || a->score_in == nullptr || a->len_in == nullptr || a->st_in == nullptr || a->ids_out == nullptr ||
      a->score_out == nullptr || a->len_out == nullptr || a->st_out == nullptr || a->parent == nullptr ||
      (a->step + 1 == a->num_steps && (a->out_ids == nullptr || a->out_len == nullptr || a->out_score == nullptr)))
    return fail(PARSEQ_ERR_INVALID_ARG, "beam_select: missing state or output array");
  if (lex && (a->edge_class == nullptr || a->edge_child == nullptr || a->terminal == nullptr || a->node_out == nullptr ||
              (a->step > 0 && a->node_in == nullptr)))
    return fail(PARSEQ_ERR_INVALID_ARG, "beam_select: incomplete lexicon");
  PQ_TRY(ensure_kernel_attributes());
  pq::BeamLex bl{};
  if (lex) bl = pq::BeamLex{a->first_edge, a->edge_class, a->edge_child, a->terminal, a->roots, a->node_in, a->node_out};
  return launch_k(g_default_opts, lex ? pq::beam_select_kernel<true> : pq::beam_select_kernel<false>,
                  dim3(static_cast<unsigned>(a->batch)), dim3(pq::BEAM_THREADS), 0, reinterpret_cast<cudaStream_t>(stream),
                  a->logits, reinterpret_cast<const float2*>(a->part),
                  reinterpret_cast<const unsigned long long*>(lex ? nullptr : a->keys), a->ntiles, static_cast<long long>(a->row0),
                  static_cast<long long>(a->img_stride), static_cast<long long>(a->slot_stride), C, K, a->step, a->num_steps,
                  a->class_mask, a->mask_ld, a->ids_in, a->score_in, a->len_in, a->st_in, a->ids_out, a->score_out, a->len_out,
                  a->st_out, a->parent, a->ids_ld, a->out_ids, a->out_len, a->out_score, bl);
}

}
```

### parseq_b200/csrc/gemm_ln.cuh

```cuda
#pragma once
#include "gemm.cuh"

namespace pq {

struct GemmLnParams {
  int M, K;
  const float* bias;
  const float* gamma;
  const float* beta;
  float eps;
  int num_m_tiles;
};

constexpr int GLN_THREADS = 384;
constexpr int GLN_BLOCK_M = 64;

template <int D, int MODE>
struct GemmLnCfg {
  static_assert(MODE == 0 || MODE == 1, "MODE");
  static constexpr int kCG = MODE == 0 ? 1 : 2;
  static constexpr int kTileM = GLN_BLOCK_M * kCG;
  static constexpr int kCols = D;
  static constexpr int kNW = kCols / 2;
  static constexpr int kParts = 2;
  static constexpr int kABox = GLN_BLOCK_M;
  static constexpr int kLoadRows = MODE == 1 ? D / 2 : kCols;
  static constexpr int kBox = kLoadRows > 256 ? kLoadRows / 2 : kLoadRows;
  static constexpr int kABytes = GLN_BLOCK_M * GEMM_BLOCK_K * 2;
  static constexpr int kBBytes = kCols * GEMM_BLOCK_K * 2;
  static constexpr int kStageBytes = kABytes + kBBytes;
  static constexpr int kParamBytes = 3 * kCols * 4 + 2 * kParts * GLN_BLOCK_M * 4;
  static constexpr int kBarBytes = 256;
  static constexpr int kStagesRaw = (232448 - 1024 - kBarBytes - kParamBytes) / kStageBytes;
  static constexpr int kStages = kStagesRaw > 6 ? 6 : kStagesRaw;
  static constexpr int kSmemBytes = kStages * kStageBytes + kParamBytes + kBarBytes + 1024;
  static_assert(D == 192 || D == 384, "embed_dim");
  static_assert(kNW % 16 == 0 && kNW <= 256, "wgmma N");
  static_assert((kNW * GEMM_BLOCK_K * 2) % 1024 == 0 && (kBox * GEMM_BLOCK_K * 2) % 1024 == 0, "1024-B aligned operand tiles");
  static_assert(kStages >= 3, "pipeline depth");
};

template <int D>
struct GemmLnCfg<D, 2> {
  static_assert(D == 384, "the persistent column-split kernel is built for D = 384");
  static constexpr int kCG = 2;
  static constexpr int kTileM = GLN_BLOCK_M;
  static constexpr int kCols = D / 2;
  static constexpr int kABox = GLN_BLOCK_M;
  static constexpr int kBox = kCols;
  static constexpr int kABytes = GLN_BLOCK_M * GEMM_BLOCK_K * 2;
  static constexpr int kBBytes = kCols * GEMM_BLOCK_K * 2;
  static constexpr int kStageBytes = kABytes + kBBytes;
  static constexpr int kStages = 3;
  static constexpr int kXBoxCols = 32;
  static constexpr int kXBoxBytes = GLN_BLOCK_M * kXBoxCols * 4;
  static constexpr int kXBytes = GLN_BLOCK_M * kCols * 4;
  static constexpr int kParamBytes = 3 * kCols * 4 + 2 * 2 * 4 * GLN_BLOCK_M * 4;
  static constexpr int kBarBytes = 256;
  static constexpr int kSmemBytes = kStages * kStageBytes + 2 * kXBytes + kParamBytes + kBarBytes + 1024;
  static_assert(kSmemBytes <= 232448, "shared memory");
};

constexpr int GLN_PARTS4_MIN_K = 768;

template <int PARTS>
__device__ __forceinline__ float gln_row_total(const float* s_part, int r) {
  float t = s_part[r] + s_part[GLN_BLOCK_M + r];
  if constexpr (PARTS == 4) t += s_part[2 * GLN_BLOCK_M + r] + s_part[3 * GLN_BLOCK_M + r];
  return t;
}

template <int D, int NW>
__device__ __forceinline__ void gln_epilogue(float (&acc)[NW / 2], float* __restrict__ x, __nv_bfloat16* __restrict__ xn, int M,
                                             float eps, int m0, int wg, const float* s_bias, const float* s_gamma,
                                             const float* s_beta, float* s_part) {
  constexpr int kNW = NW;
  const int t = threadIdx.x & 127;
  const int lane = t & 31;
  const int lr = (t >> 5) * 16 + (lane >> 2);
  const bool ok_a = m0 + lr < M, ok_b = m0 + lr + 8 < M;
  float* xa = x + static_cast<long long>(m0 + lr) * D + wg * kNW + 2 * (lane & 3);
  float* xb = xa + 8ll * D;

  float sa = 0.f, sb = 0.f;
#pragma unroll
  for (int i = 0; i < kNW / 8; ++i) {
    const int cl = wg * kNW + i * 8 + 2 * (lane & 3);
    const float b0 = s_bias[cl], b1 = s_bias[cl + 1];
    float2 xo = ok_a ? *reinterpret_cast<const float2*>(xa + i * 8) : make_float2(0.f, 0.f);
    acc[4 * i] = (acc[4 * i] + b0) + xo.x;
    acc[4 * i + 1] = (acc[4 * i + 1] + b1) + xo.y;
    if (ok_a) *reinterpret_cast<float2*>(xa + i * 8) = make_float2(acc[4 * i], acc[4 * i + 1]);
    xo = ok_b ? *reinterpret_cast<const float2*>(xb + i * 8) : make_float2(0.f, 0.f);
    acc[4 * i + 2] = (acc[4 * i + 2] + b0) + xo.x;
    acc[4 * i + 3] = (acc[4 * i + 3] + b1) + xo.y;
    if (ok_b) *reinterpret_cast<float2*>(xb + i * 8) = make_float2(acc[4 * i + 2], acc[4 * i + 3]);
    sa += acc[4 * i] + acc[4 * i + 1];
    sb += acc[4 * i + 2] + acc[4 * i + 3];
  }
  float mean_a = 0.f, mean_b = 0.f, rstd_a = 0.f, rstd_b = 0.f;
#pragma unroll
  for (int round = 0; round < 2; ++round) {
    if (round == 1) {
      sa = 0.f;
      sb = 0.f;
#pragma unroll
      for (int i = 0; i < kNW / 8; ++i) {
        const float a0 = acc[4 * i] - mean_a, a1 = acc[4 * i + 1] - mean_a;
        const float d0 = acc[4 * i + 2] - mean_b, d1 = acc[4 * i + 3] - mean_b;
        sa += a0 * a0 + a1 * a1;
        sb += d0 * d0 + d1 * d1;
      }
    }
    sa += __shfl_xor_sync(0xffffffffu, sa, 1);
    sa += __shfl_xor_sync(0xffffffffu, sa, 2);
    sb += __shfl_xor_sync(0xffffffffu, sb, 1);
    sb += __shfl_xor_sync(0xffffffffu, sb, 2);
    float* slot = s_part + (round * 2 + wg) * GLN_BLOCK_M;
    if ((lane & 3) == 0) {
      slot[lr] = sa;
      slot[lr + 8] = sb;
    }
    asm volatile("bar.sync 1, 256;" ::: "memory");
    const float* tot = s_part + round * 2 * GLN_BLOCK_M;
    const float ta = gln_row_total<2>(tot, lr), tb = gln_row_total<2>(tot, lr + 8);
    if (round == 0) {
      mean_a = ta * (1.0f / D);
      mean_b = tb * (1.0f / D);
    } else {
      rstd_a = 1.0f / sqrtf(ta * (1.0f / D) + eps);
      rstd_b = 1.0f / sqrtf(tb * (1.0f / D) + eps);
    }
  }
  uint32_t* na = reinterpret_cast<uint32_t*>(xn + static_cast<long long>(m0 + lr) * D + wg * kNW + 2 * (lane & 3));
  uint32_t* nb = na + 4ll * D;
#pragma unroll
  for (int i = 0; i < kNW / 8; ++i) {
    const int cl = wg * kNW + i * 8 + 2 * (lane & 3);
    const float g0 = s_gamma[cl], g1 = s_gamma[cl + 1], e0 = s_beta[cl], e1 = s_beta[cl + 1];
    if (ok_a) na[i * 4] = pack_bf16((acc[4 * i] - mean_a) * rstd_a * g0 + e0, (acc[4 * i + 1] - mean_a) * rstd_a * g1 + e1);
    if (ok_b) nb[i * 4] = pack_bf16((acc[4 * i + 2] - mean_b) * rstd_b * g0 + e0, (acc[4 * i + 3] - mean_b) * rstd_b * g1 + e1);
  }
}

template <int D, int PARTS>
__device__ __forceinline__ void gln_pair_epilogue(float (&acc)[D / 4], const uint8_t* xs, float* __restrict__ x,
                                                  __nv_bfloat16* __restrict__ xn, int M, float eps, int m0, int c0,
                                                  uint32_t rank, const float* s_bias, const float* s_gamma,
                                                  const float* s_beta, float* s_part, uint64_t* stat_bar, uint32_t par,
                                                  uint64_t* x_empty) {
  using Cfg = GemmLnCfg<D, 2>;
  constexpr int kI = Cfg::kCols / 8;
  constexpr int kH = PARTS / 2;
  const int t = threadIdx.x & 127;
  const int lane = t & 31;
  const int lr = (t >> 5) * 16 + (lane >> 2);
  const bool ok_a = m0 + lr < M, ok_b = m0 + lr + 8 < M;
  float* xa = x + static_cast<long long>(m0 + lr) * D + c0 + 2 * (lane & 3);
  float* xb = xa + 8ll * D;
  const uint8_t* xsa = xs + lr * 128 + (lane & 1) * 8;
  const uint8_t* xsb = xsa + 8 * 128;
  const uint32_t peer = rank ^ 1u;

  float sa[kH], sb[kH];
#pragma unroll
  for (int h = 0; h < kH; ++h) { sa[h] = 0.f; sb[h] = 0.f; }
#pragma unroll
  for (int i = 0; i < kI; ++i) {
    const int h = i / (kI / kH);
    const int cl = i * 8 + 2 * (lane & 3);
    const float b0 = s_bias[cl], b1 = s_bias[cl + 1];
    const int off = (i >> 2) * Cfg::kXBoxBytes + ((((i & 3) * 2 + ((lane >> 1) & 1)) ^ (lane >> 2)) << 4);
    float2 xo = *reinterpret_cast<const float2*>(xsa + off);
    acc[4 * i] = (acc[4 * i] + b0) + xo.x;
    acc[4 * i + 1] = (acc[4 * i + 1] + b1) + xo.y;
    if (ok_a) *reinterpret_cast<float2*>(xa + i * 8) = make_float2(acc[4 * i], acc[4 * i + 1]);
    xo = *reinterpret_cast<const float2*>(xsb + off);
    acc[4 * i + 2] = (acc[4 * i + 2] + b0) + xo.x;
    acc[4 * i + 3] = (acc[4 * i + 3] + b1) + xo.y;
    if (ok_b) *reinterpret_cast<float2*>(xb + i * 8) = make_float2(acc[4 * i + 2], acc[4 * i + 3]);
    sa[h] += acc[4 * i] + acc[4 * i + 1];
    sb[h] += acc[4 * i + 2] + acc[4 * i + 3];
  }
  mbar_arrive(x_empty);
  float mean_a = 0.f, mean_b = 0.f, rstd_a = 0.f, rstd_b = 0.f;
#pragma unroll
  for (int round = 0; round < 2; ++round) {
    if (round == 1) {
#pragma unroll
      for (int h = 0; h < kH; ++h) { sa[h] = 0.f; sb[h] = 0.f; }
#pragma unroll
      for (int i = 0; i < kI; ++i) {
        const int h = i / (kI / kH);
        const float a0 = acc[4 * i] - mean_a, a1 = acc[4 * i + 1] - mean_a;
        const float d0 = acc[4 * i + 2] - mean_b, d1 = acc[4 * i + 3] - mean_b;
        sa[h] += a0 * a0 + a1 * a1;
        sb[h] += d0 * d0 + d1 * d1;
      }
    }
    float* slots = s_part + round * PARTS * GLN_BLOCK_M;
#pragma unroll
    for (int h = 0; h < kH; ++h) {
      sa[h] += __shfl_xor_sync(0xffffffffu, sa[h], 1);
      sa[h] += __shfl_xor_sync(0xffffffffu, sa[h], 2);
      sb[h] += __shfl_xor_sync(0xffffffffu, sb[h], 1);
      sb[h] += __shfl_xor_sync(0xffffffffu, sb[h], 2);
      float* slot = slots + (static_cast<int>(rank & 1u) * kH + h) * GLN_BLOCK_M;
      if ((lane & 3) == 0) {
        slot[lr] = sa[h];
        slot[lr + 8] = sb[h];
        st_cluster_f32(mapa_cluster(smem_u32(slot + lr), peer), sa[h]);
        st_cluster_f32(mapa_cluster(smem_u32(slot + lr + 8), peer), sb[h]);
      }
    }
    mbar_arrive(&stat_bar[round]);
    mbar_arrive_cluster(mapa_cluster(smem_u32(&stat_bar[round]), peer));
    mbar_wait_cluster(&stat_bar[round], par);
    const float ta = gln_row_total<PARTS>(slots, lr), tb = gln_row_total<PARTS>(slots, lr + 8);
    if (round == 0) {
      mean_a = ta * (1.0f / D);
      mean_b = tb * (1.0f / D);
    } else {
      rstd_a = 1.0f / sqrtf(ta * (1.0f / D) + eps);
      rstd_b = 1.0f / sqrtf(tb * (1.0f / D) + eps);
    }
  }
  uint32_t* na = reinterpret_cast<uint32_t*>(xn + static_cast<long long>(m0 + lr) * D + c0 + 2 * (lane & 3));
  uint32_t* nb = na + 4ll * D;
#pragma unroll
  for (int i = 0; i < kI; ++i) {
    const int cl = i * 8 + 2 * (lane & 3);
    const float g0 = s_gamma[cl], g1 = s_gamma[cl + 1], e0 = s_beta[cl], e1 = s_beta[cl + 1];
    if (ok_a) na[i * 4] = pack_bf16((acc[4 * i] - mean_a) * rstd_a * g0 + e0, (acc[4 * i + 1] - mean_a) * rstd_a * g1 + e1);
    if (ok_b) nb[i * 4] = pack_bf16((acc[4 * i + 2] - mean_b) * rstd_b * g0 + e0, (acc[4 * i + 3] - mean_b) * rstd_b * g1 + e1);
  }
}

template <int D>
__device__ __forceinline__ void gln_pair_persistent(const CUtensorMap* tmA, const CUtensorMap* tmB, const CUtensorMap* tmX,
                                                    float* __restrict__ x, __nv_bfloat16* __restrict__ xn,
                                                    const GemmLnParams& p) {
  using Cfg = GemmLnCfg<D, 2>;
  extern __shared__ uint8_t smem_raw[];
  const uint32_t raw_addr = smem_u32(smem_raw);
  const uint32_t pad = ((raw_addr + 1023u) & ~1023u) - raw_addr;
  uint8_t* smem = smem_raw + pad;
  uint8_t* xs = smem + Cfg::kStages * Cfg::kStageBytes;
  float* s_bias = reinterpret_cast<float*>(xs + 2 * Cfg::kXBytes);
  float* s_gamma = s_bias + Cfg::kCols;
  float* s_beta = s_gamma + Cfg::kCols;
  float* s_part = s_beta + Cfg::kCols;
  uint64_t* full_bar = reinterpret_cast<uint64_t*>(reinterpret_cast<uint8_t*>(s_bias) + Cfg::kParamBytes);
  uint64_t* empty_bar = full_bar + Cfg::kStages;
  uint64_t* x_full = empty_bar + Cfg::kStages;
  uint64_t* x_empty = x_full + 2;
  uint64_t* stat_bar = x_empty + 2;

  const uint32_t rank = cluster_ctarank();
  const int cluster = static_cast<int>(blockIdx.x / Cfg::kCG), clusters = static_cast<int>(gridDim.x / Cfg::kCG);
  const int c0 = static_cast<int>(rank & 1u) * Cfg::kCols;
  const int num_kb = (p.K + GEMM_BLOCK_K - 1) / GEMM_BLOCK_K;

  grid_dep_launch();
  if (threadIdx.x == 0) {
    prefetch_tmap(tmA);
    prefetch_tmap(tmB);
    prefetch_tmap(tmX);
    for (int s = 0; s < Cfg::kStages; ++s) {
      mbar_init(&full_bar[s], 1);
      mbar_init(&empty_bar[s], 1);
    }
    for (int w = 0; w < 2; ++w) {
      mbar_init(&x_full[w], 1);
      mbar_init(&x_empty[w], 128);
    }
    for (int i = 0; i < 4; ++i) mbar_init(&stat_bar[i], 2 * 128);
    fence_mbar_init();
  }
  for (int j = threadIdx.x; j < Cfg::kCols; j += GLN_THREADS) {
    s_bias[j] = (p.bias != nullptr) ? __ldg(p.bias + c0 + j) : 0.0f;
    s_gamma[j] = __ldg(p.gamma + c0 + j);
    s_beta[j] = __ldg(p.beta + c0 + j);
  }
  cluster_sync_all();
  grid_dep_wait();

  if (threadIdx.x < 128) {
    setmaxnreg_dec<40>();
    if (threadIdx.x == 0) {
      int stage = 0;
      uint32_t phase = 0;
      int j = 0;
      for (int tile = cluster; tile < p.num_m_tiles; tile += clusters, ++j) {
        const int m0 = tile * Cfg::kTileM;
        const int w = j & 1;
        mbar_wait_mma(&x_empty[w], ((j >> 1) & 1) ^ 1u);
        mbar_expect_tx(&x_full[w], Cfg::kXBytes);
#pragma unroll
        for (int b = 0; b < Cfg::kCols / Cfg::kXBoxCols; ++b)
          tma_load_2d(xs + w * Cfg::kXBytes + b * Cfg::kXBoxBytes, tmX, &x_full[w], c0 + b * Cfg::kXBoxCols, m0);
        for (int kb = 0; kb < num_kb; ++kb) {
          mbar_wait_mma(&empty_bar[stage], phase ^ 1u);
          uint8_t* sa = smem + stage * Cfg::kStageBytes;
          mbar_expect_tx(&full_bar[stage], Cfg::kStageBytes);
          tma_load_2d(sa, tmA, &full_bar[stage], kb * GEMM_BLOCK_K, m0);
          tma_load_2d(sa + Cfg::kABytes, tmB, &full_bar[stage], kb * GEMM_BLOCK_K, c0);
          if (++stage == Cfg::kStages) { stage = 0; phase ^= 1u; }
        }
      }
    }
    __syncwarp();
  } else {
    setmaxnreg_inc<232>();
    const int wg = (threadIdx.x >> 7) - 1;
    const bool parts4 = p.K >= GLN_PARTS4_MIN_K;
    const bool leader = (threadIdx.x & 127) == 0;
    uint8_t* xw = xs + wg * Cfg::kXBytes;
    int stage = 0;
    uint32_t phase = 0, par = 0;
    if (wg == 1) ring_advance(stage, phase, num_kb, Cfg::kStages);
#pragma unroll 1
    for (int tile = cluster + wg * clusters; tile < p.num_m_tiles; tile += 2 * clusters) {
      const int m0 = tile * Cfg::kTileM;
      if (tile != cluster) named_bar_sync(1 + wg, 256);
      float acc[Cfg::kCols / 2];
#pragma unroll
      for (int i = 0; i < Cfg::kCols / 2; ++i) acc[i] = 0.0f;
      int prev = -1;
#pragma unroll 1
      for (int kb = 0; kb < num_kb; ++kb) {
        mbar_wait_mma(&full_bar[stage], phase);
        const uint32_t base = smem_u32(smem + stage * Cfg::kStageBytes);
        const uint64_t da = make_desc_k_sw128(base);
        const uint64_t db = make_desc_k_sw128(base + Cfg::kABytes);
        wgmma_fence();
#pragma unroll
        for (int k = 0; k < GEMM_BLOCK_K / 16; ++k)
          wgmma_bf16<Cfg::kCols>(acc, da + static_cast<uint64_t>(2 * k), db + static_cast<uint64_t>(2 * k),
                                 static_cast<uint32_t>((kb | k) != 0));
        wgmma_commit();
        if (prev >= 0) {
          wgmma_wait<1>();
          if (leader) mbar_arrive(&empty_bar[prev]);
        }
        prev = stage;
        if (++stage == Cfg::kStages) { stage = 0; phase ^= 1u; }
      }
      if (tile + clusters < p.num_m_tiles) named_bar_arrive(1 + (wg ^ 1), 256);
      wgmma_wait<0>();
      wgmma_reg_fence(acc);
      if (leader) mbar_arrive(&empty_bar[prev]);
      ring_advance(stage, phase, num_kb, Cfg::kStages);
      mbar_wait_mma(&x_full[wg], par);
      if (parts4)
        gln_pair_epilogue<D, 4>(acc, xw, x, xn, p.M, p.eps, m0, c0, rank, s_bias, s_gamma, s_beta,
                                s_part + wg * 2 * 4 * GLN_BLOCK_M, stat_bar + 2 * wg, par, &x_empty[wg]);
      else
        gln_pair_epilogue<D, 2>(acc, xw, x, xn, p.M, p.eps, m0, c0, rank, s_bias, s_gamma, s_beta,
                                s_part + wg * 2 * 4 * GLN_BLOCK_M, stat_bar + 2 * wg, par, &x_empty[wg]);
      par ^= 1u;
    }
  }
  cluster_sync_all();
}

template <int D, int MODE>
__global__ void __launch_bounds__(GLN_THREADS, 1)
gemm_ln_fused_kernel(const __grid_constant__ CUtensorMap tmA, const __grid_constant__ CUtensorMap tmB,
                     const __grid_constant__ CUtensorMap tmX, float* __restrict__ x, __nv_bfloat16* __restrict__ xn,
                     const GemmLnParams p) {
  if constexpr (MODE == 2) {
    gln_pair_persistent<D>(&tmA, &tmB, &tmX, x, xn, p);
  } else {
    using Cfg = GemmLnCfg<D, MODE>;
    constexpr int kNW = Cfg::kNW;
    extern __shared__ uint8_t smem_raw[];
    const uint32_t raw_addr = smem_u32(smem_raw);
    const uint32_t pad = ((raw_addr + 1023u) & ~1023u) - raw_addr;
    uint8_t* smem = smem_raw + pad;
    float* s_bias = reinterpret_cast<float*>(smem + Cfg::kStages * Cfg::kStageBytes);
    float* s_gamma = s_bias + Cfg::kCols;
    float* s_beta = s_gamma + Cfg::kCols;
    float* s_part = s_beta + Cfg::kCols;
    uint64_t* full_bar = reinterpret_cast<uint64_t*>(reinterpret_cast<uint8_t*>(s_bias) + Cfg::kParamBytes);
    uint64_t* empty_bar = full_bar + Cfg::kStages;

    const uint32_t rank = (MODE == 1) ? cluster_ctarank() : 0u;
    const int cluster = blockIdx.x / Cfg::kCG;
    const int m0 = cluster * Cfg::kTileM + static_cast<int>(rank) * GLN_BLOCK_M;
    const int num_kb = (p.K + GEMM_BLOCK_K - 1) / GEMM_BLOCK_K;

    grid_dep_launch();
    if (threadIdx.x == 0) {
      prefetch_tmap(&tmA);
      prefetch_tmap(&tmB);
      for (int s = 0; s < Cfg::kStages; ++s) {
        mbar_init(&full_bar[s], 1);
        mbar_init(&empty_bar[s], MODE == 1 ? 4 : 2);
      }
      fence_mbar_init();
    }
    for (int j = threadIdx.x; j < Cfg::kCols; j += GLN_THREADS) {
      s_bias[j] = (p.bias != nullptr) ? __ldg(p.bias + j) : 0.0f;
      s_gamma[j] = __ldg(p.gamma + j);
      s_beta[j] = __ldg(p.beta + j);
    }
    if constexpr (MODE == 1) cluster_sync_all(); else __syncthreads();
    grid_dep_wait();

    if (threadIdx.x < 128) {
      if (threadIdx.x == 0) {
        int stage = 0;
        uint32_t phase = 0;
        for (int kb = 0; kb < num_kb; ++kb) {
          mbar_wait_mma(&empty_bar[stage], phase ^ 1u);
          uint8_t* sa = smem + stage * Cfg::kStageBytes;
          uint8_t* sb = sa + Cfg::kABytes;
          mbar_expect_tx(&full_bar[stage], Cfg::kStageBytes);
          tma_load_2d(sa, &tmA, &full_bar[stage], kb * GEMM_BLOCK_K, m0);
          if constexpr (MODE == 1) {
            const int r = static_cast<int>(rank);
            tma_load_2d_mcast(sb + r * Cfg::kLoadRows * GEMM_BLOCK_K * 2, &tmB, &full_bar[stage], kb * GEMM_BLOCK_K,
                              r * Cfg::kLoadRows, 0x3);
          } else {
#pragma unroll
            for (int b = 0; b < Cfg::kLoadRows / Cfg::kBox; ++b)
              tma_load_2d(sb + b * Cfg::kBox * GEMM_BLOCK_K * 2, &tmB, &full_bar[stage], kb * GEMM_BLOCK_K, b * Cfg::kBox);
          }
          if (++stage == Cfg::kStages) { stage = 0; phase ^= 1u; }
        }
      }
      __syncwarp();
    } else {
      const int wg = (threadIdx.x >> 7) - 1;
      float acc[kNW / 2];
#pragma unroll
      for (int i = 0; i < kNW / 2; ++i) acc[i] = 0.0f;
      int stage = 0;
      uint32_t phase = 0;
      wg_mainloop<kNW, MODE == 1>(acc, smem, Cfg::kStageBytes, 0, Cfg::kABytes + wg * kNW * GEMM_BLOCK_K * 2, full_bar,
                                  empty_bar, Cfg::kStages, num_kb, stage, phase);
      gln_epilogue<D, kNW>(acc, x, xn, p.M, p.eps, m0, wg, s_bias, s_gamma, s_beta, s_part);
    }
    if constexpr (MODE == 1) cluster_sync_all();
  }
}

}
```

### parseq_b200/csrc/ptx.cuh

```cuda
#pragma once
#include <cuda_bf16.h>
#include <cuda_runtime.h>
#include <stdint.h>

namespace pq {

__device__ __forceinline__ uint32_t smem_u32(const void* p) {
  return static_cast<uint32_t>(__cvta_generic_to_shared(p));
}
__device__ __forceinline__ uint32_t lane_id() { return threadIdx.x & 31u; }

constexpr int ARGMAX_NONE = 0x7fffffff;
__device__ __forceinline__ bool argmax_better(float v, int j, float best, int bi) {
  if (j == ARGMAX_NONE) return false;
  if (bi == ARGMAX_NONE) return true;
  const bool vn = isnan(v), bn = isnan(best);
  if (vn != bn) return vn;
  if (vn || v == best) return j < bi;
  return v > best;
}
__device__ __forceinline__ void argmax_fold(float& best, int& bi, float v, int j) {
  if (argmax_better(v, j, best, bi)) { best = v; bi = j; }
}
__device__ __forceinline__ void argmax_shfl(float& best, int& bi, int lo = 1, int hi = 32) {
#pragma unroll
  for (int o = lo; o < hi; o <<= 1) {
    const float ov = __shfl_xor_sync(0xffffffffu, best, o);
    const int oi = __shfl_xor_sync(0xffffffffu, bi, o);
    argmax_fold(best, bi, ov, oi);
  }
}
__device__ __forceinline__ void argmax_scan(float& best, int& bi, float v, int j) {
  if (v > best) { best = v; bi = j; }
}
__device__ __forceinline__ int argmax_finish(float best, int bi, const float* row, int n, int lane) {
  argmax_shfl(best, bi);
  int first_nan = ARGMAX_NONE;
  for (int j = lane; j < n; j += 32)
    if (isnan(row[j])) { first_nan = j; break; }
  first_nan = __reduce_min_sync(0xffffffffu, first_nan);
  if (first_nan != ARGMAX_NONE) return first_nan;
  return bi == ARGMAX_NONE ? 0 : bi;
}
__device__ __forceinline__ bool class_allowed(const uint32_t* row, int c) {
  return c == 0 || ((__ldg(row + (c >> 5)) >> (c & 31)) & 1u);
}
__device__ __forceinline__ int class_mask_words(int C) { return (C + 31) >> 5; }
constexpr int BEAM_TOPK_LD = 16;
__device__ __forceinline__ unsigned long long beam_order_key(float x, int c) {
  uint32_t o;
  if (isnan(x)) {
    o = 0xffffffffu;
  } else {
    const uint32_t u = __float_as_uint(x == 0.0f ? 0.0f : x);
    o = (u & 0x80000000u) ? ~u : (u | 0x80000000u);
  }
  return (static_cast<unsigned long long>(o) << 32) | (0xffffffffu - static_cast<uint32_t>(c));
}
__device__ __forceinline__ float beam_key_value(unsigned long long key) {
  const uint32_t o = static_cast<uint32_t>(key >> 32);
  if (o == 0xffffffffu) return __int_as_float(0x7fffffff);
  return __uint_as_float((o & 0x80000000u) ? (o & 0x7fffffffu) : ~o);
}
__device__ __forceinline__ int beam_key_class(unsigned long long key) {
  return static_cast<int>(0xffffffffu - static_cast<uint32_t>(key));
}


__device__ __forceinline__ void mbar_init(uint64_t* bar, uint32_t count) {
  asm volatile("mbarrier.init.shared::cta.b64 [%0], %1;" ::"r"(smem_u32(bar)), "r"(count) : "memory");
}
__device__ __forceinline__ void fence_mbar_init() {
  asm volatile("fence.mbarrier_init.release.cluster;" ::: "memory");
}
__device__ __forceinline__ void mbar_expect_tx(uint64_t* bar, uint32_t bytes) {
  asm volatile("mbarrier.arrive.expect_tx.shared::cta.b64 _, [%0], %1;" ::"r"(smem_u32(bar)), "r"(bytes)
               : "memory");
}
__device__ __forceinline__ void mbar_arrive(uint64_t* bar) {
  asm volatile("mbarrier.arrive.shared::cta.b64 _, [%0];" ::"r"(smem_u32(bar)) : "memory");
}
__device__ __forceinline__ bool mbar_try_wait(uint64_t* bar, uint32_t parity) {
  uint32_t ok;
  asm volatile(
      "{\n\t.reg .pred p;\n\t"
      "mbarrier.try_wait.parity.shared::cta.b64 p, [%1], %2;\n\t"
      "selp.b32 %0, 1, 0, p;\n\t}"
      : "=r"(ok)
      : "r"(smem_u32(bar)), "r"(parity)
      : "memory");
  return ok != 0;
}
#ifndef PQ_SPIN_LIMIT_CYCLES
#define PQ_SPIN_LIMIT_CYCLES (4000000000ll)
#endif
__device__ __forceinline__ void mbar_wait(uint64_t* bar, uint32_t parity) {
  if (mbar_try_wait(bar, parity)) return;
  long long t0 = clock64();
  uint32_t it = 0;
  while (!mbar_try_wait(bar, parity)) {
    if (((++it) & 0x3ffu) == 0 && (clock64() - t0) > PQ_SPIN_LIMIT_CYCLES) {
      printf("[parseq_b200] mbarrier wait timeout: block %d thread %d bar %u parity %u\n", blockIdx.x,
             threadIdx.x, smem_u32(bar), parity);
      __trap();
    }
  }
}

__device__ __forceinline__ void mbar_wait_mma(uint64_t* bar, uint32_t parity) {
  if (mbar_try_wait(bar, parity)) return;
  long long t0 = clock64();
  uint32_t it = 0;
  while (!mbar_try_wait(bar, parity))
    if (((++it) & 0x3ffu) == 0 && (clock64() - t0) > PQ_SPIN_LIMIT_CYCLES) __trap();
}

__device__ __forceinline__ void grid_dep_launch() { asm volatile("griddepcontrol.launch_dependents;" ::: "memory"); }
__device__ __forceinline__ void grid_dep_wait() { asm volatile("griddepcontrol.wait;" ::: "memory"); }

__device__ __forceinline__ void named_bar_sync(int id, int count) {
  asm volatile("bar.sync %0, %1;" ::"r"(id), "r"(count) : "memory");
}
__device__ __forceinline__ void named_bar_arrive(int id, int count) {
  asm volatile("bar.arrive %0, %1;" ::"r"(id), "r"(count) : "memory");
}
template <int N>
__device__ __forceinline__ void setmaxnreg_dec() { asm volatile("setmaxnreg.dec.sync.aligned.u32 %0;" ::"n"(N)); }
template <int N>
__device__ __forceinline__ void setmaxnreg_inc() { asm volatile("setmaxnreg.inc.sync.aligned.u32 %0;" ::"n"(N)); }

__device__ __forceinline__ uint32_t cluster_ctarank() {
  uint32_t r;
  asm volatile("mov.u32 %0, %%cluster_ctarank;" : "=r"(r));
  return r;
}
__device__ __forceinline__ void cluster_sync_all() {
  asm volatile("barrier.cluster.arrive.release.aligned;\n\tbarrier.cluster.wait.acquire.aligned;" ::: "memory");
}
__device__ __forceinline__ uint32_t mapa_cluster(uint32_t local_smem_addr, uint32_t rank) {
  uint32_t r;
  asm volatile("mapa.shared::cluster.u32 %0, %1, %2;" : "=r"(r) : "r"(local_smem_addr), "r"(rank));
  return r;
}
__device__ __forceinline__ void mbar_arrive_cluster(uint32_t cluster_addr) {
  asm volatile("mbarrier.arrive.release.cluster.shared::cluster.b64 _, [%0];" ::"r"(cluster_addr) : "memory");
}

__device__ __forceinline__ void prefetch_tmap(const void* tmap) {
  asm volatile("prefetch.tensormap [%0];" ::"l"(reinterpret_cast<uint64_t>(tmap)) : "memory");
}
__device__ __forceinline__ void tma_load_2d(void* smem_dst, const void* tmap, uint64_t* bar, int32_t c0,
                                            int32_t c1) {
  asm volatile(
      "cp.async.bulk.tensor.2d.shared::cluster.global.mbarrier::complete_tx::bytes [%0], [%1, {%3, %4}], [%2];"
      ::"r"(smem_u32(smem_dst)), "l"(reinterpret_cast<uint64_t>(tmap)), "r"(smem_u32(bar)), "r"(c0), "r"(c1)
      : "memory");
}

__device__ __forceinline__ void tma_load_3d(void* smem_dst, const void* tmap, uint64_t* bar, int32_t c0, int32_t c1,
                                            int32_t c2) {
  asm volatile(
      "cp.async.bulk.tensor.3d.shared::cluster.global.mbarrier::complete_tx::bytes [%0], [%1, {%3, %4, %5}], [%2];"
      ::"r"(smem_u32(smem_dst)), "l"(reinterpret_cast<uint64_t>(tmap)), "r"(smem_u32(bar)), "r"(c0), "r"(c1), "r"(c2)
      : "memory");
}

__device__ __forceinline__ void tma_load_4d(void* smem_dst, const void* tmap, uint64_t* bar, int32_t c0, int32_t c1,
                                            int32_t c2, int32_t c3) {
  asm volatile(
      "cp.async.bulk.tensor.4d.shared::cluster.global.mbarrier::complete_tx::bytes [%0], [%1, {%3, %4, %5, %6}], [%2];"
      ::"r"(smem_u32(smem_dst)), "l"(reinterpret_cast<uint64_t>(tmap)), "r"(smem_u32(bar)), "r"(c0), "r"(c1), "r"(c2),
        "r"(c3)
      : "memory");
}

__device__ __forceinline__ void tma_store_2d(const void* tmap, const void* smem_src, int32_t c0, int32_t c1) {
  asm volatile("cp.async.bulk.tensor.2d.global.shared::cta.bulk_group [%0, {%2, %3}], [%1];"
               ::"l"(reinterpret_cast<uint64_t>(tmap)), "r"(smem_u32(smem_src)), "r"(c0), "r"(c1)
               : "memory");
}
__device__ __forceinline__ void tma_store_3d(const void* tmap, const void* smem_src, int32_t c0, int32_t c1, int32_t c2) {
  asm volatile("cp.async.bulk.tensor.3d.global.shared::cta.bulk_group [%0, {%2, %3, %4}], [%1];"
               ::"l"(reinterpret_cast<uint64_t>(tmap)), "r"(smem_u32(smem_src)), "r"(c0), "r"(c1), "r"(c2)
               : "memory");
}
__device__ __forceinline__ void tma_reduce_add_2d(const void* tmap, const void* smem_src, int32_t c0, int32_t c1) {
  asm volatile("cp.reduce.async.bulk.tensor.2d.global.shared::cta.add.tile.bulk_group [%0, {%2, %3}], [%1];"
               ::"l"(reinterpret_cast<uint64_t>(tmap)), "r"(smem_u32(smem_src)), "r"(c0), "r"(c1)
               : "memory");
}
__device__ __forceinline__ void bulk_commit_group() { asm volatile("cp.async.bulk.commit_group;" ::: "memory"); }
template <int N>
__device__ __forceinline__ void bulk_wait_group_read() {
  asm volatile("cp.async.bulk.wait_group.read %0;" ::"n"(N) : "memory");
}
template <int N>
__device__ __forceinline__ void bulk_wait_group() {
  asm volatile("cp.async.bulk.wait_group %0;" ::"n"(N) : "memory");
}
__device__ __forceinline__ void fence_proxy_async_smem() { asm volatile("fence.proxy.async.shared::cta;" ::: "memory"); }

__device__ __forceinline__ void tma_load_2d_mcast(void* smem_dst, const void* tmap, uint64_t* bar, int32_t c0, int32_t c1,
                                                  uint16_t cta_mask) {
  asm volatile(
      "cp.async.bulk.tensor.2d.shared::cluster.global.mbarrier::complete_tx::bytes.multicast::cluster [%0], [%1, {%3, %4}], [%2], %5;"
      ::"r"(smem_u32(smem_dst)), "l"(reinterpret_cast<uint64_t>(tmap)), "r"(smem_u32(bar)), "r"(c0), "r"(c1), "h"(cta_mask)
      : "memory");
}
__device__ __forceinline__ void mbar_wait_cluster(uint64_t* bar, uint32_t parity) {
  uint32_t ok = 0;
  long long t0 = clock64();
  uint32_t it = 0;
  while (true) {
    asm volatile(
        "{\n\t.reg .pred p;\n\t"
        "mbarrier.try_wait.parity.acquire.cluster.shared::cta.b64 p, [%1], %2;\n\t"
        "selp.b32 %0, 1, 0, p;\n\t}"
        : "=r"(ok)
        : "r"(smem_u32(bar)), "r"(parity)
        : "memory");
    if (ok) return;
    if (((++it) & 0x3ffu) == 0 && (clock64() - t0) > PQ_SPIN_LIMIT_CYCLES) __trap();
  }
}
__device__ __forceinline__ void st_cluster_f32(uint32_t cluster_addr, float v) {
  asm volatile("st.shared::cluster.f32 [%0], %1;" ::"r"(cluster_addr), "f"(v) : "memory");
}

__device__ __forceinline__ uint64_t make_desc_k_sw128(uint32_t smem_addr) {
  uint64_t d = 0;
  d |= static_cast<uint64_t>((smem_addr >> 4) & 0x3FFFu);
  d |= static_cast<uint64_t>(1u) << 16;
  d |= static_cast<uint64_t>(1024u >> 4) << 32;
  d |= static_cast<uint64_t>(1u) << 62;
  return d;
}
__device__ __forceinline__ void wgmma_fence() { asm volatile("wgmma.fence.sync.aligned;" ::: "memory"); }
__device__ __forceinline__ void wgmma_commit() { asm volatile("wgmma.commit_group.sync.aligned;" ::: "memory"); }
template <int N>
__device__ __forceinline__ void wgmma_wait() { asm volatile("wgmma.wait_group.sync.aligned %0;" ::"n"(N) : "memory"); }
template <int R>
__device__ __forceinline__ void wgmma_reg_fence(float (&d)[R]) {
#pragma unroll
  for (int i = 0; i < R; ++i) asm volatile("" : "+f"(d[i])::"memory");
}

template <int N>
__device__ __forceinline__ void wgmma_bf16(float (&d)[N / 2], uint64_t da, uint64_t db, uint32_t accumulate);
template <>
__device__ __forceinline__ void wgmma_bf16<32>(float (&d)[16], uint64_t da, uint64_t db, uint32_t accumulate) {
  asm volatile(
      "{\n\t.reg .pred p;\n\tsetp.ne.b32 p, %18, 0;\n\t"
      "wgmma.mma_async.sync.aligned.m64n32k16.f32.bf16.bf16 {%0, %1, %2, %3, %4, %5, %6, %7, %8, %9, %10, %11, %12, %13, %14, %15}, %16, %17, p, 1, 1, 0, 0;\n\t}"
      : "+f"(d[0]), "+f"(d[1]), "+f"(d[2]), "+f"(d[3]), "+f"(d[4]), "+f"(d[5]), "+f"(d[6]), "+f"(d[7]), "+f"(d[8]), "+f"(d[9]), "+f"(d[10]), "+f"(d[11]), "+f"(d[12]), "+f"(d[13]), "+f"(d[14]), "+f"(d[15])
      : "l"(da), "l"(db), "r"(accumulate));
}
template <>
__device__ __forceinline__ void wgmma_bf16<64>(float (&d)[32], uint64_t da, uint64_t db, uint32_t accumulate) {
  asm volatile(
      "{\n\t.reg .pred p;\n\tsetp.ne.b32 p, %34, 0;\n\t"
      "wgmma.mma_async.sync.aligned.m64n64k16.f32.bf16.bf16 {%0, %1, %2, %3, %4, %5, %6, %7, %8, %9, %10, %11, %12, %13, %14, %15, %16, %17, %18, %19, %20, %21, %22, %23, %24, %25, %26, %27, %28, %29, %30, %31}, %32, %33, p, 1, 1, 0, 0;\n\t}"
      : "+f"(d[0]), "+f"(d[1]), "+f"(d[2]), "+f"(d[3]), "+f"(d[4]), "+f"(d[5]), "+f"(d[6]), "+f"(d[7]), "+f"(d[8]), "+f"(d[9]), "+f"(d[10]), "+f"(d[11]), "+f"(d[12]), "+f"(d[13]), "+f"(d[14]), "+f"(d[15]), "+f"(d[16]), "+f"(d[17]), "+f"(d[18]), "+f"(d[19]), "+f"(d[20]), "+f"(d[21]), "+f"(d[22]), "+f"(d[23]), "+f"(d[24]), "+f"(d[25]), "+f"(d[26]), "+f"(d[27]), "+f"(d[28]), "+f"(d[29]), "+f"(d[30]), "+f"(d[31])
      : "l"(da), "l"(db), "r"(accumulate));
}
template <>
__device__ __forceinline__ void wgmma_bf16<96>(float (&d)[48], uint64_t da, uint64_t db, uint32_t accumulate) {
  asm volatile(
      "{\n\t.reg .pred p;\n\tsetp.ne.b32 p, %50, 0;\n\t"
      "wgmma.mma_async.sync.aligned.m64n96k16.f32.bf16.bf16 {%0, %1, %2, %3, %4, %5, %6, %7, %8, %9, %10, %11, %12, %13, %14, %15, %16, %17, %18, %19, %20, %21, %22, %23, %24, %25, %26, %27, %28, %29, %30, %31, %32, %33, %34, %35, %36, %37, %38, %39, %40, %41, %42, %43, %44, %45, %46, %47}, %48, %49, p, 1, 1, 0, 0;\n\t}"
      : "+f"(d[0]), "+f"(d[1]), "+f"(d[2]), "+f"(d[3]), "+f"(d[4]), "+f"(d[5]), "+f"(d[6]), "+f"(d[7]), "+f"(d[8]), "+f"(d[9]), "+f"(d[10]), "+f"(d[11]), "+f"(d[12]), "+f"(d[13]), "+f"(d[14]), "+f"(d[15]), "+f"(d[16]), "+f"(d[17]), "+f"(d[18]), "+f"(d[19]), "+f"(d[20]), "+f"(d[21]), "+f"(d[22]), "+f"(d[23]), "+f"(d[24]), "+f"(d[25]), "+f"(d[26]), "+f"(d[27]), "+f"(d[28]), "+f"(d[29]), "+f"(d[30]), "+f"(d[31]), "+f"(d[32]), "+f"(d[33]), "+f"(d[34]), "+f"(d[35]), "+f"(d[36]), "+f"(d[37]), "+f"(d[38]), "+f"(d[39]), "+f"(d[40]), "+f"(d[41]), "+f"(d[42]), "+f"(d[43]), "+f"(d[44]), "+f"(d[45]), "+f"(d[46]), "+f"(d[47])
      : "l"(da), "l"(db), "r"(accumulate));
}
template <>
__device__ __forceinline__ void wgmma_bf16<128>(float (&d)[64], uint64_t da, uint64_t db, uint32_t accumulate) {
  asm volatile(
      "{\n\t.reg .pred p;\n\tsetp.ne.b32 p, %66, 0;\n\t"
      "wgmma.mma_async.sync.aligned.m64n128k16.f32.bf16.bf16 {%0, %1, %2, %3, %4, %5, %6, %7, %8, %9, %10, %11, %12, %13, %14, %15, %16, %17, %18, %19, %20, %21, %22, %23, %24, %25, %26, %27, %28, %29, %30, %31, %32, %33, %34, %35, %36, %37, %38, %39, %40, %41, %42, %43, %44, %45, %46, %47, %48, %49, %50, %51, %52, %53, %54, %55, %56, %57, %58, %59, %60, %61, %62, %63}, %64, %65, p, 1, 1, 0, 0;\n\t}"
      : "+f"(d[0]), "+f"(d[1]), "+f"(d[2]), "+f"(d[3]), "+f"(d[4]), "+f"(d[5]), "+f"(d[6]), "+f"(d[7]), "+f"(d[8]), "+f"(d[9]), "+f"(d[10]), "+f"(d[11]), "+f"(d[12]), "+f"(d[13]), "+f"(d[14]), "+f"(d[15]), "+f"(d[16]), "+f"(d[17]), "+f"(d[18]), "+f"(d[19]), "+f"(d[20]), "+f"(d[21]), "+f"(d[22]), "+f"(d[23]), "+f"(d[24]), "+f"(d[25]), "+f"(d[26]), "+f"(d[27]), "+f"(d[28]), "+f"(d[29]), "+f"(d[30]), "+f"(d[31]), "+f"(d[32]), "+f"(d[33]), "+f"(d[34]), "+f"(d[35]), "+f"(d[36]), "+f"(d[37]), "+f"(d[38]), "+f"(d[39]), "+f"(d[40]), "+f"(d[41]), "+f"(d[42]), "+f"(d[43]), "+f"(d[44]), "+f"(d[45]), "+f"(d[46]), "+f"(d[47]), "+f"(d[48]), "+f"(d[49]), "+f"(d[50]), "+f"(d[51]), "+f"(d[52]), "+f"(d[53]), "+f"(d[54]), "+f"(d[55]), "+f"(d[56]), "+f"(d[57]), "+f"(d[58]), "+f"(d[59]), "+f"(d[60]), "+f"(d[61]), "+f"(d[62]), "+f"(d[63])
      : "l"(da), "l"(db), "r"(accumulate));
}
template <>
__device__ __forceinline__ void wgmma_bf16<192>(float (&d)[96], uint64_t da, uint64_t db, uint32_t accumulate) {
  asm volatile(
      "{\n\t.reg .pred p;\n\tsetp.ne.b32 p, %98, 0;\n\t"
      "wgmma.mma_async.sync.aligned.m64n192k16.f32.bf16.bf16 {%0, %1, %2, %3, %4, %5, %6, %7, %8, %9, %10, %11, %12, %13, %14, %15, %16, %17, %18, %19, %20, %21, %22, %23, %24, %25, %26, %27, %28, %29, %30, %31, %32, %33, %34, %35, %36, %37, %38, %39, %40, %41, %42, %43, %44, %45, %46, %47, %48, %49, %50, %51, %52, %53, %54, %55, %56, %57, %58, %59, %60, %61, %62, %63, %64, %65, %66, %67, %68, %69, %70, %71, %72, %73, %74, %75, %76, %77, %78, %79, %80, %81, %82, %83, %84, %85, %86, %87, %88, %89, %90, %91, %92, %93, %94, %95}, %96, %97, p, 1, 1, 0, 0;\n\t}"
      : "+f"(d[0]), "+f"(d[1]), "+f"(d[2]), "+f"(d[3]), "+f"(d[4]), "+f"(d[5]), "+f"(d[6]), "+f"(d[7]), "+f"(d[8]), "+f"(d[9]), "+f"(d[10]), "+f"(d[11]), "+f"(d[12]), "+f"(d[13]), "+f"(d[14]), "+f"(d[15]), "+f"(d[16]), "+f"(d[17]), "+f"(d[18]), "+f"(d[19]), "+f"(d[20]), "+f"(d[21]), "+f"(d[22]), "+f"(d[23]), "+f"(d[24]), "+f"(d[25]), "+f"(d[26]), "+f"(d[27]), "+f"(d[28]), "+f"(d[29]), "+f"(d[30]), "+f"(d[31]), "+f"(d[32]), "+f"(d[33]), "+f"(d[34]), "+f"(d[35]), "+f"(d[36]), "+f"(d[37]), "+f"(d[38]), "+f"(d[39]), "+f"(d[40]), "+f"(d[41]), "+f"(d[42]), "+f"(d[43]), "+f"(d[44]), "+f"(d[45]), "+f"(d[46]), "+f"(d[47]), "+f"(d[48]), "+f"(d[49]), "+f"(d[50]), "+f"(d[51]), "+f"(d[52]), "+f"(d[53]), "+f"(d[54]), "+f"(d[55]), "+f"(d[56]), "+f"(d[57]), "+f"(d[58]), "+f"(d[59]), "+f"(d[60]), "+f"(d[61]), "+f"(d[62]), "+f"(d[63]), "+f"(d[64]), "+f"(d[65]), "+f"(d[66]), "+f"(d[67]), "+f"(d[68]), "+f"(d[69]), "+f"(d[70]), "+f"(d[71]), "+f"(d[72]), "+f"(d[73]), "+f"(d[74]), "+f"(d[75]), "+f"(d[76]), "+f"(d[77]), "+f"(d[78]), "+f"(d[79]), "+f"(d[80]), "+f"(d[81]), "+f"(d[82]), "+f"(d[83]), "+f"(d[84]), "+f"(d[85]), "+f"(d[86]), "+f"(d[87]), "+f"(d[88]), "+f"(d[89]), "+f"(d[90]), "+f"(d[91]), "+f"(d[92]), "+f"(d[93]), "+f"(d[94]), "+f"(d[95])
      : "l"(da), "l"(db), "r"(accumulate));
}
template <>
__device__ __forceinline__ void wgmma_bf16<256>(float (&d)[128], uint64_t da, uint64_t db, uint32_t accumulate) {
  asm volatile(
      "{\n\t.reg .pred p;\n\tsetp.ne.b32 p, %130, 0;\n\t"
      "wgmma.mma_async.sync.aligned.m64n256k16.f32.bf16.bf16 {%0, %1, %2, %3, %4, %5, %6, %7, %8, %9, %10, %11, %12, %13, %14, %15, %16, %17, %18, %19, %20, %21, %22, %23, %24, %25, %26, %27, %28, %29, %30, %31, %32, %33, %34, %35, %36, %37, %38, %39, %40, %41, %42, %43, %44, %45, %46, %47, %48, %49, %50, %51, %52, %53, %54, %55, %56, %57, %58, %59, %60, %61, %62, %63, %64, %65, %66, %67, %68, %69, %70, %71, %72, %73, %74, %75, %76, %77, %78, %79, %80, %81, %82, %83, %84, %85, %86, %87, %88, %89, %90, %91, %92, %93, %94, %95, %96, %97, %98, %99, %100, %101, %102, %103, %104, %105, %106, %107, %108, %109, %110, %111, %112, %113, %114, %115, %116, %117, %118, %119, %120, %121, %122, %123, %124, %125, %126, %127}, %128, %129, p, 1, 1, 0, 0;\n\t}"
      : "+f"(d[0]), "+f"(d[1]), "+f"(d[2]), "+f"(d[3]), "+f"(d[4]), "+f"(d[5]), "+f"(d[6]), "+f"(d[7]), "+f"(d[8]), "+f"(d[9]), "+f"(d[10]), "+f"(d[11]), "+f"(d[12]), "+f"(d[13]), "+f"(d[14]), "+f"(d[15]), "+f"(d[16]), "+f"(d[17]), "+f"(d[18]), "+f"(d[19]), "+f"(d[20]), "+f"(d[21]), "+f"(d[22]), "+f"(d[23]), "+f"(d[24]), "+f"(d[25]), "+f"(d[26]), "+f"(d[27]), "+f"(d[28]), "+f"(d[29]), "+f"(d[30]), "+f"(d[31]), "+f"(d[32]), "+f"(d[33]), "+f"(d[34]), "+f"(d[35]), "+f"(d[36]), "+f"(d[37]), "+f"(d[38]), "+f"(d[39]), "+f"(d[40]), "+f"(d[41]), "+f"(d[42]), "+f"(d[43]), "+f"(d[44]), "+f"(d[45]), "+f"(d[46]), "+f"(d[47]), "+f"(d[48]), "+f"(d[49]), "+f"(d[50]), "+f"(d[51]), "+f"(d[52]), "+f"(d[53]), "+f"(d[54]), "+f"(d[55]), "+f"(d[56]), "+f"(d[57]), "+f"(d[58]), "+f"(d[59]), "+f"(d[60]), "+f"(d[61]), "+f"(d[62]), "+f"(d[63]), "+f"(d[64]), "+f"(d[65]), "+f"(d[66]), "+f"(d[67]), "+f"(d[68]), "+f"(d[69]), "+f"(d[70]), "+f"(d[71]), "+f"(d[72]), "+f"(d[73]), "+f"(d[74]), "+f"(d[75]), "+f"(d[76]), "+f"(d[77]), "+f"(d[78]), "+f"(d[79]), "+f"(d[80]), "+f"(d[81]), "+f"(d[82]), "+f"(d[83]), "+f"(d[84]), "+f"(d[85]), "+f"(d[86]), "+f"(d[87]), "+f"(d[88]), "+f"(d[89]), "+f"(d[90]), "+f"(d[91]), "+f"(d[92]), "+f"(d[93]), "+f"(d[94]), "+f"(d[95]), "+f"(d[96]), "+f"(d[97]), "+f"(d[98]), "+f"(d[99]), "+f"(d[100]), "+f"(d[101]), "+f"(d[102]), "+f"(d[103]), "+f"(d[104]), "+f"(d[105]), "+f"(d[106]), "+f"(d[107]), "+f"(d[108]), "+f"(d[109]), "+f"(d[110]), "+f"(d[111]), "+f"(d[112]), "+f"(d[113]), "+f"(d[114]), "+f"(d[115]), "+f"(d[116]), "+f"(d[117]), "+f"(d[118]), "+f"(d[119]), "+f"(d[120]), "+f"(d[121]), "+f"(d[122]), "+f"(d[123]), "+f"(d[124]), "+f"(d[125]), "+f"(d[126]), "+f"(d[127])
      : "l"(da), "l"(db), "r"(accumulate));
}

__device__ __forceinline__ void ldmatrix_x4(uint32_t addr, uint32_t& r0, uint32_t& r1, uint32_t& r2, uint32_t& r3) {
  asm volatile("ldmatrix.sync.aligned.m8n8.x4.shared.b16 {%0, %1, %2, %3}, [%4];"
               : "=r"(r0), "=r"(r1), "=r"(r2), "=r"(r3)
               : "r"(addr));
}
__device__ __forceinline__ void ldmatrix_x4_trans(uint32_t addr, uint32_t& r0, uint32_t& r1, uint32_t& r2,
                                                  uint32_t& r3) {
  asm volatile("ldmatrix.sync.aligned.m8n8.x4.trans.shared.b16 {%0, %1, %2, %3}, [%4];"
               : "=r"(r0), "=r"(r1), "=r"(r2), "=r"(r3)
               : "r"(addr));
}
__device__ __forceinline__ void mma_bf16_16816(float (&d)[4], uint32_t a0, uint32_t a1, uint32_t a2, uint32_t a3,
                                               uint32_t b0, uint32_t b1) {
  asm volatile(
      "mma.sync.aligned.m16n8k16.row.col.f32.bf16.bf16.f32 {%0, %1, %2, %3}, {%4, %5, %6, %7}, {%8, %9}, "
      "{%0, %1, %2, %3};"
      : "+f"(d[0]), "+f"(d[1]), "+f"(d[2]), "+f"(d[3])
      : "r"(a0), "r"(a1), "r"(a2), "r"(a3), "r"(b0), "r"(b1));
}
__device__ __forceinline__ void cp_async_16(uint32_t smem_dst, const void* gsrc) {
  asm volatile("cp.async.cg.shared.global [%0], [%1], 16;" ::"r"(smem_dst), "l"(gsrc) : "memory");
}
__device__ __forceinline__ void cp_async_wait_all() { asm volatile("cp.async.wait_all;" ::: "memory"); }

__device__ __forceinline__ long long blocked_off(long long rows_total, long long row, int col) {
  return (static_cast<long long>(col >> 6) * rows_total + row) * 64 + (col & 63);
}

__device__ __forceinline__ uint32_t pack_bf16(float lo, float hi) {
  __nv_bfloat162 v = __floats2bfloat162_rn(lo, hi);
  return *reinterpret_cast<uint32_t*>(&v);
}
__device__ __forceinline__ float ex2_approx(float x) {
  float y;
  asm("ex2.approx.ftz.f32 %0, %1;" : "=f"(y) : "f"(x));
  return y;
}
__device__ __forceinline__ float gelu_erf(float x) {
  const float u = fminf(fabsf(x), 8.5f);
  const float t = fmaf(u, 2.0f / 8.5f, -1.0f);
  float q = 8.503329848e-03f;
  q = fmaf(q, t, -2.785826938e-02f);
  q = fmaf(q, t, 4.857975011e-02f);
  q = fmaf(q, t, -8.378244194e-02f);
  q = fmaf(q, t, 1.570760869e-01f);
  q = fmaf(q, t, -2.896217881e-01f);
  q = fmaf(q, t, -1.247551552e+01f);
  q = fmaf(q, t, -2.737368526e+01f);
  q = fmaf(q, t, -1.651358203e+01f);
  const float h = ex2_approx(q);
  return fmaf(-u, h, fmaxf(x, 0.0f));
}

}
```

### parseq_b200/engine.py

```python
from __future__ import annotations

import ctypes as C
import os
from typing import Dict, Optional

from .build import LIB_PATH

_lib = None


class ParseqConfigC(C.Structure):
    _fields_ = [(n, C.c_int32) for n in (
        "img_h", "img_w", "patch_h", "patch_w", "embed_dim", "enc_num_heads", "enc_mlp_ratio", "enc_depth",
        "dec_num_heads", "dec_mlp_ratio", "dec_depth", "max_label_length", "num_tokens", "max_batch", "device", "arch")]


class ForwardArgsC(C.Structure):
    _fields_ = [("batch", C.c_int32), ("max_length", C.c_int32), ("decode_ar", C.c_int32),
                ("refine_iters", C.c_int32), ("forced_ids", C.c_void_p), ("forced_refine", C.c_void_p),
                ("class_mask", C.c_void_p), ("attn_maps", C.c_void_p)]


class CropsC(C.Structure):
    _fields_ = [("data", C.c_void_p), ("data_bytes", C.c_int64), ("offsets", C.c_void_p), ("sizes", C.c_void_p),
                ("rotation", C.c_int32), ("rotations", C.c_void_p)]


class OrientArgsC(C.Structure):
    _fields_ = [("num_orientations", C.c_int32), ("orientations", C.c_int32 * 4), ("min_confidence", C.c_float),
                ("rotation_out", C.c_void_p), ("confidence_out", C.c_void_p)]


def orient_args(orientations, min_confidence, rotation_ptr, confidence_ptr) -> OrientArgsC:
    o = list(orientations)
    return OrientArgsC(len(o), (C.c_int32 * 4)(*(o + [0] * (4 - len(o)))[:4]),
                       float("nan") if min_confidence is None else float(min_confidence), rotation_ptr, confidence_ptr)


class ScoreArgsC(C.Structure):
    _fields_ = [("batch", C.c_int32), ("num_candidates", C.c_int32), ("per_image", C.c_void_p), ("targets", C.c_void_p),
                ("lengths", C.c_void_p), ("attn_maps", C.c_void_p)]


class BeamArgsC(C.Structure):
    _fields_ = [("batch", C.c_int32), ("beam_width", C.c_int32), ("max_length", C.c_int32), ("class_mask", C.c_void_p),
                ("attn_maps", C.c_void_p)]


class LexiconDescC(C.Structure):
    _fields_ = [("num_nodes", C.c_int32), ("num_edges", C.c_int32), ("first_edge", C.c_void_p), ("edge_class", C.c_void_p),
                ("edge_child", C.c_void_p), ("terminal", C.c_void_p)]


class BeamSelectArgsC(C.Structure):
    _fields_ = [("logits", C.c_void_p), ("part", C.c_void_p), ("keys", C.c_void_p), ("ntiles", C.c_int32),
                ("row0", C.c_int64), ("img_stride", C.c_int64), ("slot_stride", C.c_int64),
                ("batch", C.c_int32), ("num_classes", C.c_int32), ("beam_width", C.c_int32), ("step", C.c_int32),
                ("num_steps", C.c_int32), ("class_mask", C.c_void_p), ("mask_ld", C.c_int32),
                ("ids_in", C.c_void_p), ("score_in", C.c_void_p), ("len_in", C.c_void_p), ("st_in", C.c_void_p),
                ("ids_out", C.c_void_p), ("score_out", C.c_void_p), ("len_out", C.c_void_p), ("st_out", C.c_void_p),
                ("parent", C.c_void_p), ("ids_ld", C.c_int32), ("out_ids", C.c_void_p), ("out_len", C.c_void_p),
                ("out_score", C.c_void_p), ("first_edge", C.c_void_p), ("edge_class", C.c_void_p),
                ("edge_child", C.c_void_p), ("terminal", C.c_void_p), ("roots", C.c_void_p), ("node_in", C.c_void_p),
                ("node_out", C.c_void_p)]


def lexicon_desc(first_edge, edge_class, edge_child, terminal) -> LexiconDescC:
    return LexiconDescC(int(terminal.shape[0]), int(edge_class.shape[0]), first_edge.ctypes.data, edge_class.ctypes.data,
                        edge_child.ctypes.data, terminal.ctypes.data)


class LexiconHandle:

    def __init__(self, lib, ptr):
        self.lib, self.ptr = lib, ptr

    def __del__(self):
        try:
            if self.ptr:
                self.lib.parseq_lexicon_destroy(self.ptr)
                self.ptr = None
        except Exception:
            pass


EXPORTS = [
    "parseq_create", "parseq_destroy", "parseq_set_weight", "parseq_num_weights", "parseq_weight_key",
    "parseq_finalize", "parseq_forward", "parseq_forward_host", "parseq_forward_u8", "parseq_forward_host_u8",
    "parseq_resize_crops", "parseq_forward_crops", "parseq_forward_host_crops", "parseq_forward_crops_oriented",
    "parseq_score", "parseq_score_u8", "parseq_score_check", "parseq_beam_search", "parseq_beam_search_u8",
    "parseq_lexicon_check", "parseq_lexicon_create", "parseq_lexicon_destroy", "parseq_beam_search_lexicon",
    "parseq_beam_search_lexicon_u8",
    "parseq_postprocess", "parseq_encode", "parseq_decode", "parseq_decode_ex", "parseq_head", "parseq_text_embed", "parseq_kernel_launches", "parseq_debug_int", "parseq_bench_tma_stream",
    "parseq_set_option", "parseq_get_timing", "parseq_get_ar_profile", "parseq_last_error", "parseq_version", "parseq_gemm_bf16", "parseq_gemm_ln_bf16", "parseq_mlp_ln_bf16", "parseq_layernorm_bf16",
    "parseq_enc_attention", "parseq_qkv_attention_bf16", "parseq_head_lse_bf16", "parseq_head_topk_bf16",
    "parseq_beam_select",
]


def load_library(path: Optional[str] = None):
    global _lib
    if _lib is not None and path is None:
        return _lib
    p = path or os.environ.get("PARSEQ_B200_LIB", LIB_PATH)
    if not os.path.exists(p):
        raise RuntimeError(f"{p} not found: build it with `python -m parseq_b200.build` "
                           "(there is no CPU / PyTorch fallback)")
    lib = C.CDLL(p)
    lib.parseq_last_error.restype = C.c_char_p
    lib.parseq_version.restype = C.c_char_p
    lib.parseq_weight_key.restype = C.c_char_p
    lib.parseq_weight_key.argtypes = [C.c_void_p, C.c_int, C.POINTER(C.c_int64)]
    lib.parseq_bench_tma_stream.argtypes = [C.c_void_p, C.c_int64, C.c_int, C.c_int, C.c_int, C.c_int, C.c_int, C.c_void_p, C.c_void_p]
    lib.parseq_debug_int.restype = C.c_int64
    lib.parseq_debug_int.argtypes = [C.c_void_p, C.c_char_p]
    lib.parseq_kernel_launches.restype = C.c_int64
    lib.parseq_kernel_launches.argtypes = [C.c_void_p]
    lib.parseq_create.argtypes = [C.POINTER(ParseqConfigC), C.POINTER(C.c_void_p)]
    lib.parseq_destroy.argtypes = [C.c_void_p]
    lib.parseq_destroy.restype = None
    lib.parseq_set_weight.argtypes = [C.c_void_p, C.c_char_p, C.c_void_p, C.c_int64]
    lib.parseq_num_weights.argtypes = [C.c_void_p]
    lib.parseq_finalize.argtypes = [C.c_void_p, C.c_void_p]
    lib.parseq_forward.argtypes = [C.c_void_p, C.POINTER(ForwardArgsC), C.c_void_p, C.c_void_p, C.c_void_p,
                                   C.c_void_p, C.c_void_p]
    lib.parseq_forward_host.argtypes = lib.parseq_forward.argtypes
    lib.parseq_forward_u8.argtypes = lib.parseq_forward.argtypes
    lib.parseq_forward_host_u8.argtypes = lib.parseq_forward.argtypes
    lib.parseq_resize_crops.argtypes = [C.c_void_p, C.c_int32, C.POINTER(CropsC), C.c_void_p, C.c_void_p]
    lib.parseq_forward_crops.argtypes = [C.c_void_p, C.POINTER(ForwardArgsC), C.POINTER(CropsC), C.c_void_p, C.c_void_p,
                                         C.c_void_p, C.c_void_p]
    lib.parseq_forward_host_crops.argtypes = lib.parseq_forward_crops.argtypes
    lib.parseq_forward_crops_oriented.argtypes = [C.c_void_p, C.POINTER(ForwardArgsC), C.POINTER(CropsC),
                                                  C.POINTER(OrientArgsC), C.c_void_p, C.c_void_p, C.c_void_p, C.c_void_p]
    lib.parseq_score.argtypes = [C.c_void_p, C.POINTER(ScoreArgsC), C.c_void_p, C.c_void_p, C.c_void_p, C.c_void_p]
    lib.parseq_score_u8.argtypes = lib.parseq_score.argtypes
    lib.parseq_score_check.argtypes = [C.POINTER(ParseqConfigC), C.POINTER(ScoreArgsC)]
    lib.parseq_beam_search.argtypes = [C.c_void_p, C.POINTER(BeamArgsC), C.c_void_p, C.c_void_p, C.c_void_p, C.c_void_p,
                                       C.c_void_p]
    lib.parseq_beam_search_u8.argtypes = lib.parseq_beam_search.argtypes
    lib.parseq_lexicon_check.argtypes = [C.POINTER(ParseqConfigC), C.POINTER(LexiconDescC)]
    lib.parseq_lexicon_create.argtypes = [C.c_void_p, C.POINTER(LexiconDescC), C.POINTER(C.c_void_p), C.c_void_p]
    lib.parseq_lexicon_destroy.argtypes = [C.c_void_p]
    lib.parseq_lexicon_destroy.restype = None
    lib.parseq_beam_search_lexicon.argtypes = [C.c_void_p, C.POINTER(BeamArgsC), C.c_void_p, C.c_void_p, C.c_void_p,
                                               C.c_void_p, C.c_void_p, C.c_void_p, C.c_void_p]
    lib.parseq_beam_search_lexicon_u8.argtypes = lib.parseq_beam_search_lexicon.argtypes
    lib.parseq_postprocess.argtypes = [C.c_void_p, C.c_int32, C.c_int32, C.c_int32, C.c_int32, C.c_void_p, C.c_void_p,
                                       C.c_void_p, C.c_void_p]
    lib.parseq_encode.argtypes = [C.c_void_p, C.c_int32, C.c_void_p, C.c_void_p, C.c_void_p]
    lib.parseq_decode.argtypes = [C.c_void_p, C.c_int32, C.c_int32, C.c_int32, C.c_void_p, C.c_void_p, C.c_void_p, C.c_void_p,
                                  C.c_void_p, C.c_void_p, C.c_void_p]
    lib.parseq_decode_ex.argtypes = [C.c_void_p, C.c_int32, C.c_int32, C.c_int32, C.c_void_p, C.c_void_p, C.c_void_p, C.c_void_p,
                                     C.c_void_p, C.c_void_p, C.c_void_p, C.c_void_p]
    lib.parseq_head.argtypes = [C.c_void_p, C.c_int32, C.c_void_p, C.c_void_p, C.c_void_p]
    lib.parseq_text_embed.argtypes = [C.c_void_p, C.c_int32, C.c_void_p, C.c_void_p, C.c_void_p]
    lib.parseq_set_option.argtypes = [C.c_void_p, C.c_char_p, C.c_int64]
    lib.parseq_get_timing.argtypes = [C.c_void_p, C.c_int, C.POINTER(C.c_double), C.POINTER(C.c_double),
                                      C.POINTER(C.c_int64)]
    lib.parseq_gemm_bf16.argtypes = [C.c_void_p, C.c_int64, C.c_void_p, C.c_int64, C.c_void_p, C.c_int, C.c_int,
                                     C.c_int, C.c_int, C.c_float, C.c_void_p, C.c_int64, C.c_int, C.c_void_p,
                                     C.c_int64, C.c_void_p]
    lib.parseq_gemm_ln_bf16.argtypes = [C.c_void_p, C.c_int64, C.c_void_p, C.c_int64, C.c_void_p, C.c_int, C.c_int, C.c_int,
                                        C.c_void_p, C.c_void_p, C.c_void_p, C.c_float, C.c_void_p, C.c_void_p]
    lib.parseq_mlp_ln_bf16.argtypes = [C.c_void_p, C.c_void_p, C.c_void_p, C.c_void_p, C.c_void_p, C.c_int, C.c_int, C.c_void_p,
                                       C.c_void_p, C.c_void_p, C.c_float, C.c_void_p, C.c_void_p]
    lib.parseq_layernorm_bf16.argtypes = [C.c_void_p, C.c_void_p, C.c_void_p, C.c_float, C.c_int, C.c_int,
                                          C.c_void_p, C.c_void_p, C.c_void_p]
    lib.parseq_enc_attention.argtypes = [C.c_void_p, C.c_int, C.c_int, C.c_int, C.c_int, C.c_void_p, C.c_void_p]
    lib.parseq_qkv_attention_bf16.argtypes = [C.c_void_p, C.c_void_p, C.c_void_p, C.c_int, C.c_int, C.c_int, C.c_int,
                                              C.c_void_p, C.c_void_p]
    lib.parseq_head_lse_bf16.argtypes = [C.c_void_p, C.c_int64, C.c_void_p, C.c_int64, C.c_void_p, C.c_int, C.c_int, C.c_int,
                                         C.c_void_p, C.c_void_p, C.c_void_p, C.c_void_p]
    lib.parseq_head_topk_bf16.argtypes = [C.c_void_p, C.c_int64, C.c_void_p, C.c_int64, C.c_void_p, C.c_int, C.c_int, C.c_int,
                                          C.c_int, C.c_void_p, C.c_int, C.c_void_p, C.c_void_p, C.c_void_p]
    lib.parseq_beam_select.argtypes = [C.POINTER(BeamSelectArgsC), C.c_void_p]
    if path is None:
        _lib = lib
    return lib


class EngineError(RuntimeError):
    pass


def check(lib, rc: int):
    if rc != 0:
        raise EngineError(f"parseq_b200 error {rc}: {lib.parseq_last_error().decode()}")


def config_c(cfg, device: int = 0, max_batch: int = 0) -> ParseqConfigC:
    return ParseqConfigC(cfg.img_size[0], cfg.img_size[1], cfg.patch_size[0], cfg.patch_size[1], cfg.embed_dim,
                         cfg.enc_num_heads, cfg.enc_mlp_ratio, cfg.enc_depth, cfg.dec_num_heads, cfg.dec_mlp_ratio,
                         cfg.dec_depth, cfg.max_label_length, cfg.num_tokens, max_batch, device,
                         1 if getattr(cfg, "arch", "parseq") == "vitstr" else 0)


class Engine:

    def __init__(self, cfg, device: int = 0, max_batch: int = 0):
        self.lib = load_library()
        self.cfg = cfg
        c = config_c(cfg, device, max_batch)
        h = C.c_void_p()
        check(self.lib, self.lib.parseq_create(C.byref(c), C.byref(h)))
        self.handle = h
        self.device = device

    def close(self):
        if getattr(self, "handle", None):
            self.lib.parseq_destroy(self.handle)
            self.handle = None

    def __del__(self):
        try:
            self.close()
        except Exception:
            pass

    def weight_keys(self) -> Dict[str, int]:
        out = {}
        n = self.lib.parseq_num_weights(self.handle)
        for i in range(n):
            numel = C.c_int64()
            k = self.lib.parseq_weight_key(self.handle, i, C.byref(numel))
            out[k.decode()] = numel.value
        return out

    def load_state_dict(self, sd, stream: int = 0):
        import torch
        expected = self.weight_keys()
        missing = [k for k in expected if k not in sd]
        unexpected = [k for k in sd if k not in expected]
        if missing or unexpected:
            raise EngineError(f"state_dict mismatch: missing {missing[:4]}... unexpected {unexpected[:4]}...")
        for k, numel in expected.items():
            t = sd[k].detach().to(device="cpu", dtype=torch.float32).contiguous()
            if t.numel() != numel:
                raise EngineError(f"size mismatch for {k}: {tuple(t.shape)} vs {numel} elements")
            check(self.lib, self.lib.parseq_set_weight(self.handle, k.encode(), t.data_ptr(), numel))
        check(self.lib, self.lib.parseq_finalize(self.handle, stream))

    def set_option(self, name: str, value: int):
        check(self.lib, self.lib.parseq_set_option(self.handle, name.encode(), int(value)))

    TIMING_CATEGORIES = ("enc_gemm", "enc_attn", "layernorm", "dec_gemm", "dec_attn", "other", "enc_gemm_ln", "dec_ar",
                         "score_tail", "beam_select", "attn_maps", "orient")

    def get_timing(self):
        out = {}
        for i, name in enumerate(self.TIMING_CATEGORIES):
            ms, fl, n = C.c_double(), C.c_double(), C.c_int64()
            check(self.lib, self.lib.parseq_get_timing(self.handle, i, C.byref(ms), C.byref(fl), C.byref(n)))
            out[name] = dict(ms=ms.value, flops=fl.value, launches=n.value)
        return out

    def get_ar_profile(self):
        buf = (C.c_uint64 * 512)()
        self.lib.parseq_get_ar_profile.argtypes = [C.c_void_p, C.POINTER(C.c_uint64)]
        check(self.lib, self.lib.parseq_get_ar_profile(self.handle, buf))
        return [[buf[s * 16 + k] for k in range(16)] for s in range(32)]

    def debug_int(self, name: str) -> int:
        return int(self.lib.parseq_debug_int(self.handle, name.encode()))

    @property
    def launches(self) -> int:
        return int(self.lib.parseq_kernel_launches(self.handle))

    def num_steps(self, max_length) -> int:
        ml = self.cfg.max_label_length if max_length is None else min(int(max_length), self.cfg.max_label_length)
        return ml + 1

    def _args(self, batch, max_length, decode_ar, refine_iters, forced_ids=None, forced_refine=None, class_mask=None,
              attn_maps=None):
        return ForwardArgsC(batch, -1 if max_length is None else int(max_length), int(bool(decode_ar)),
                            int(refine_iters), forced_ids, forced_refine, class_mask, attn_maps)

    def forward(self, images_ptr, batch, logits_ptr, ids_ptr, steps_ptr, stream, max_length=None, decode_ar=True,
                refine_iters=1, forced_ids_ptr=None, forced_refine_ptr=None, class_mask_ptr=None, attn_maps_ptr=None):
        a = self._args(batch, max_length, decode_ar, refine_iters, forced_ids_ptr, forced_refine_ptr, class_mask_ptr,
                       attn_maps_ptr)
        check(self.lib, self.lib.parseq_forward(self.handle, C.byref(a), images_ptr, logits_ptr, ids_ptr, steps_ptr,
                                                stream))

    def forward_host(self, images_ptr, batch, logits_ptr, ids_ptr, steps_ptr, stream, max_length=None,
                     decode_ar=True, refine_iters=1, class_mask_ptr=None, attn_maps_ptr=None):
        a = self._args(batch, max_length, decode_ar, refine_iters, class_mask=class_mask_ptr, attn_maps=attn_maps_ptr)
        check(self.lib, self.lib.parseq_forward_host(self.handle, C.byref(a), images_ptr, logits_ptr, ids_ptr,
                                                     steps_ptr, stream))

    def forward_u8(self, images_ptr, batch, logits_ptr, ids_ptr, steps_ptr, stream, max_length=None, decode_ar=True,
                   refine_iters=1, host=False, class_mask_ptr=None, attn_maps_ptr=None):
        a = self._args(batch, max_length, decode_ar, refine_iters, class_mask=class_mask_ptr, attn_maps=attn_maps_ptr)
        fn = self.lib.parseq_forward_host_u8 if host else self.lib.parseq_forward_u8
        check(self.lib, fn(self.handle, C.byref(a), images_ptr, logits_ptr, ids_ptr, steps_ptr, stream))

    def resize_crops(self, crops: CropsC, batch, out_ptr, stream):
        check(self.lib, self.lib.parseq_resize_crops(self.handle, batch, C.byref(crops), out_ptr, stream))

    def forward_crops(self, crops: CropsC, batch, logits_ptr, ids_ptr, steps_ptr, stream, max_length=None, decode_ar=True,
                      refine_iters=1, host=False, class_mask_ptr=None, attn_maps_ptr=None):
        a = self._args(batch, max_length, decode_ar, refine_iters, class_mask=class_mask_ptr, attn_maps=attn_maps_ptr)
        fn = self.lib.parseq_forward_host_crops if host else self.lib.parseq_forward_crops
        check(self.lib, fn(self.handle, C.byref(a), C.byref(crops), logits_ptr, ids_ptr, steps_ptr, stream))

    def forward_crops_oriented(self, crops: CropsC, batch, orientations, min_confidence, logits_ptr, ids_ptr, steps_ptr,
                               rotation_ptr, confidence_ptr, stream, max_length=None, decode_ar=True, refine_iters=1,
                               class_mask_ptr=None, attn_maps_ptr=None):
        a = self._args(batch, max_length, decode_ar, refine_iters, class_mask=class_mask_ptr, attn_maps=attn_maps_ptr)
        o = orient_args(orientations, min_confidence, rotation_ptr, confidence_ptr)
        check(self.lib, self.lib.parseq_forward_crops_oriented(self.handle, C.byref(a), C.byref(crops), C.byref(o),
                                                               logits_ptr, ids_ptr, steps_ptr, stream))

    def score(self, images_ptr, batch, per_image, targets, lengths, scores_ptr, token_lp_ptr, stream, u8=False,
              attn_maps_ptr=None):
        a = ScoreArgsC(batch, int(targets.shape[0]), per_image.data_ptr(), targets.data_ptr(), lengths.data_ptr(),
                       attn_maps_ptr)
        fn = self.lib.parseq_score_u8 if u8 else self.lib.parseq_score
        check(self.lib, fn(self.handle, C.byref(a), images_ptr, scores_ptr, token_lp_ptr, stream))

    def beam_search(self, images_ptr, batch, beam_width, ids_ptr, lengths_ptr, scores_ptr, stream, max_length=None,
                    class_mask_ptr=None, u8=False, lexicon=None, roots=None, attn_maps_ptr=None):
        a = BeamArgsC(batch, int(beam_width), -1 if max_length is None else int(max_length), class_mask_ptr,
                      attn_maps_ptr)
        if lexicon is None:
            fn = self.lib.parseq_beam_search_u8 if u8 else self.lib.parseq_beam_search
            check(self.lib, fn(self.handle, C.byref(a), images_ptr, ids_ptr, lengths_ptr, scores_ptr, stream))
            return
        fn = self.lib.parseq_beam_search_lexicon_u8 if u8 else self.lib.parseq_beam_search_lexicon
        check(self.lib, fn(self.handle, C.byref(a), lexicon.ptr, roots.data_ptr() if roots is not None else None,
                           images_ptr, ids_ptr, lengths_ptr, scores_ptr, stream))

    def lexicon_create(self, first_edge, edge_class, edge_child, terminal, stream) -> LexiconHandle:
        d = lexicon_desc(first_edge, edge_class, edge_child, terminal)
        h = C.c_void_p()
        check(self.lib, self.lib.parseq_lexicon_create(self.handle, C.byref(d), C.byref(h), stream))
        return LexiconHandle(self.lib, h)

    def postprocess(self, logits_ptr, batch, num_steps, ids_ptr, lengths_ptr, conf_ptr, stream, eos_id=0):
        check(self.lib, self.lib.parseq_postprocess(logits_ptr, batch, num_steps, self.cfg.num_classes, eos_id, ids_ptr,
                                                    lengths_ptr, conf_ptr, stream))

    def encode(self, images_ptr, batch, memory_ptr, stream):
        check(self.lib, self.lib.parseq_encode(self.handle, batch, images_ptr, memory_ptr, stream))

    def decode(self, batch, ctx_len, num_queries, tgt_ptr, memory_ptr, query_ptr, qmask_ptr, pmask_ptr, out_ptr, stream,
               cmask_ptr=None):
        check(self.lib, self.lib.parseq_decode_ex(self.handle, batch, ctx_len, num_queries, tgt_ptr, memory_ptr, query_ptr,
                                                  qmask_ptr, pmask_ptr, cmask_ptr, out_ptr, stream))

    def head(self, rows, x_ptr, logits_ptr, stream):
        check(self.lib, self.lib.parseq_head(self.handle, rows, x_ptr, logits_ptr, stream))

    def text_embed(self, n, ids_ptr, out_ptr, stream):
        check(self.lib, self.lib.parseq_text_embed(self.handle, n, ids_ptr, out_ptr, stream))
```

Measured before the change: 41400.

## Share weight tiles across both warpgroups in gemm+LN and use st.async stats exchange

Adds a MODE 3 persistent gemm+LayerNorm kernel for D=384 and K>=768. Each stage loads one 128-row A tile and one weight slice, and both warpgroups consume it, halving weight traffic per row. The cross-CTA row-statistics exchange now uses st.async with mbarrier complete_tx instead of remote stores plus a cluster arrive/wait. A globaltimer phase profiling kernel and API are also added. The risk is that the warpgroups no longer alternate tiles, so overlap between epilogue and MMA may drop, and the X loads are now issued mid K-loop.

```diff
diff --git a/include/parseq_b200.h b/include/parseq_b200.h
--- a/include/parseq_b200.h
+++ b/include/parseq_b200.h
@@ -158,6 +158,9 @@
 int parseq_gemm_ln_bf16(const void* A, int64_t lda, const void* W, int64_t ldw, const float* bias,
                         int M, int D, int K, float* x_inout, const float* gamma, const float* beta,
                         float eps, void* xn_bf16, parseq_stream_t stream);
+int parseq_gemm_ln_profile(const void* A, int64_t lda, const void* W, int64_t ldw, const float* bias, int M, int K,
+                           float* x_inout, const float* gamma, const float* beta, float eps, void* xn_bf16,
+                           uint64_t* prof_dev, parseq_stream_t stream);
 int parseq_mlp_ln_bf16(const void* xn, const void* W1, const float* b1, const void* W2, const float* b2,
                        int M, int D, float* x_inout, const float* gamma, const float* beta, float eps,
                        void* xn_out_bf16, parseq_stream_t stream);
diff --git a/parseq_b200/csrc/engine.cu b/parseq_b200/csrc/engine.cu
--- a/parseq_b200/csrc/engine.cu
+++ b/parseq_b200/csrc/engine.cu
@@ -253,7 +253,12 @@
 }
 
 template <int D, int MODE>
-int gemm_ln_attr() { return set_smem(pq::gemm_ln_fused_kernel<D, MODE>, pq::GemmLnCfg<D, MODE>::kSmemBytes); }
+constexpr auto gemm_ln_kernel() {
+  if constexpr (MODE == 3) return pq::gemm_ln_shared_w_kernel<D>;
+  else return pq::gemm_ln_fused_kernel<D, MODE>;
+}
+template <int D, int MODE>
+int gemm_ln_attr() { return set_smem(gemm_ln_kernel<D, MODE>(), pq::GemmLnCfg<D, MODE>::kSmemBytes); }
 template <int D, int CG>
 int mlp_ln_attr() { return set_smem(pq::mlp_ln_fused_kernel<D, CG>, pq::MlpLnCfg<D, CG>::kSmemBytes); }
 template <int NK>
@@ -280,6 +285,9 @@
   PQ_TRY(set_smem(pq::dec_ln_head_argmax_kernel<768>, 226 * 1024));
   PQ_TRY((gemm_ln_attr<192, 0>())); PQ_TRY((gemm_ln_attr<384, 0>())); PQ_TRY((gemm_ln_attr<192, 1>()));
   PQ_TRY((gemm_ln_attr<384, 1>())); PQ_TRY((gemm_ln_attr<384, 2>()));
+  PQ_TRY((gemm_ln_attr<384, 3>()));
+  PQ_TRY(set_smem(pq::gemm_ln_prof_kernel<384, 2>, pq::GemmLnCfg<384, 2>::kSmemBytes));
+  PQ_TRY(set_smem(pq::gemm_ln_prof_kernel<384, 3>, pq::GemmLnCfg<384, 3>::kSmemBytes));
   PQ_TRY((mlp_ln_attr<192, 1>())); PQ_TRY((mlp_ln_attr<384, 1>())); PQ_TRY((mlp_ln_attr<192, 2>())); PQ_TRY((mlp_ln_attr<384, 2>()));
   PQ_TRY((attn_wgmma_attr<128>())); PQ_TRY((attn_wgmma_attr<256>()));
   PQ_TRY((qkv_attn_attr<192>())); PQ_TRY((qkv_attn_attr<384>()));
@@ -400,9 +408,10 @@
 }
 
 bool gemm_ln_supported(int D) { return D == 192 || D == 384; }
-template <int D, int MODE>
+template <int D, int MODE, bool PROF = false>
 int launch_gemm_ln(LaunchOpts& lo, const void* A, long long lda, const void* W, long long ldw, const float* bias, int M, int K, float* x,
-                   const float* gamma, const float* beta, float eps, void* xn, cudaStream_t st) {
+                   const float* gamma, const float* beta, float eps, void* xn, cudaStream_t st,
+                   unsigned long long* prof = nullptr) {
   using Cfg = pq::GemmLnCfg<D, MODE>;
   CUtensorMap ta, tb, tx;
   PQ_TRY(make_tmap(&ta, A, 2, M, K, lda, pq::GEMM_BLOCK_K, Cfg::kABox));
@@ -413,29 +422,35 @@
   p.M = M; p.K = K; p.bias = bias; p.gamma = gamma; p.beta = beta; p.eps = eps;
   p.num_m_tiles = (M + Cfg::kTileM - 1) / Cfg::kTileM;
   int clusters = p.num_m_tiles;
-  if constexpr (MODE == 2) {
+  if constexpr (MODE >= 2) {
     PQ_TRY(make_tmap(&tx, x, 4, M, D, D, Cfg::kXBoxCols, pq::GLN_BLOCK_M));
     if (lo.ln_clusters == 0) {
       const LaunchConfig occ(dim3(static_cast<unsigned>(lo.sm_count / Cfg::kCG * Cfg::kCG)), dim3(pq::GLN_THREADS),
                              Cfg::kSmemBytes, st, Cfg::kCG, false);
-      PQ_CUDA(cudaOccupancyMaxActiveClusters(&lo.ln_clusters, pq::gemm_ln_fused_kernel<D, MODE>, &occ.cfg));
+      PQ_CUDA(cudaOccupancyMaxActiveClusters(&lo.ln_clusters, gemm_ln_kernel<D, MODE>(), &occ.cfg));
       if (lo.ln_clusters <= 0) return fail(PARSEQ_ERR_CUDA, "gemm_ln: no cluster of the persistent kernel fits the device");
     }
     clusters = std::min(p.num_m_tiles, lo.ln_clusters);
   } else {
     tx = ta;
   }
-  return launch_ex(LaunchConfig(dim3(static_cast<unsigned>(clusters * Cfg::kCG)), dim3(pq::GLN_THREADS), Cfg::kSmemBytes, st,
-                                Cfg::kCG, cluster_pdl(lo, Cfg::kCG)),
-                   pq::gemm_ln_fused_kernel<D, MODE>, ta, tb, tx, x, reinterpret_cast<__nv_bfloat16*>(xn), p);
+  const LaunchConfig lc(dim3(static_cast<unsigned>(clusters * Cfg::kCG)), dim3(pq::GLN_THREADS), Cfg::kSmemBytes, st, Cfg::kCG,
+                        cluster_pdl(lo, Cfg::kCG));
+  if constexpr (PROF) {
+    static_assert(MODE >= 2, "the phase profile is built for MODE 2 / 3");
+    return launch_ex(lc, pq::gemm_ln_prof_kernel<D, MODE>, ta, tb, tx, x, reinterpret_cast<__nv_bfloat16*>(xn), p, prof);
+  }
+  return launch_ex(lc, gemm_ln_kernel<D, MODE>(), ta, tb, tx, x, reinterpret_cast<__nv_bfloat16*>(xn), p);
 }
 int gemm_ln_launch(LaunchOpts& lo, const void* A, long long lda, const void* W, long long ldw, const float* bias, int M, int D,
                    int K, float* x, const float* gamma, const float* beta, float eps, void* xn, cudaStream_t st) {
   if (M <= 0 || K <= 0) return fail(PARSEQ_ERR_INVALID_ARG, "gemm_ln: empty problem");
   PQ_TRY(ensure_sm_count(lo));
   PQ_TRY(load_driver_api());
-  if (D == 384 && lo.ln_split != 1)
+  if (D == 384 && lo.ln_split != 1) {
+    if (K >= pq::GLN_SHARED_W_MIN_K) return launch_gemm_ln<384, 3>(lo, A, lda, W, ldw, bias, M, K, x, gamma, beta, eps, xn, st);
     return launch_gemm_ln<384, 2>(lo, A, lda, W, ldw, bias, M, K, x, gamma, beta, eps, xn, st);
+  }
   if (lo.ln_cta_group == 2) {
     if (D == 384) return launch_gemm_ln<384, 1>(lo, A, lda, W, ldw, bias, M, K, x, gamma, beta, eps, xn, st);
     if (D == 192) return launch_gemm_ln<192, 1>(lo, A, lda, W, ldw, bias, M, K, x, gamma, beta, eps, xn, st);
@@ -3044,6 +3059,19 @@
   PQ_TRY(ensure_kernel_attributes());
   return gemm_ln_launch(g_default_opts, A, lda, W, ldw, bias, M, D, K, x_inout, gamma, beta, eps, xn_bf16, reinterpret_cast<cudaStream_t>(stream));
 }
+int parseq_gemm_ln_profile(const void* A, int64_t lda, const void* W, int64_t ldw, const float* bias, int M, int K,
+                           float* x_inout, const float* gamma, const float* beta, float eps, void* xn_bf16,
+                           uint64_t* prof_dev, parseq_stream_t stream) {
+  if (M <= 0 || K <= 0 || prof_dev == nullptr) return fail(PARSEQ_ERR_INVALID_ARG, "gemm_ln_profile: empty problem or no buffer");
+  PQ_TRY(ensure_kernel_attributes());
+  PQ_TRY(ensure_sm_count(g_default_opts));
+  PQ_TRY(load_driver_api());
+  auto* prof = reinterpret_cast<unsigned long long*>(prof_dev);
+  const cudaStream_t st = reinterpret_cast<cudaStream_t>(stream);
+  if (K >= pq::GLN_SHARED_W_MIN_K)
+    return launch_gemm_ln<384, 3, true>(g_default_opts, A, lda, W, ldw, bias, M, K, x_inout, gamma, beta, eps, xn_bf16, st, prof);
+  return launch_gemm_ln<384, 2, true>(g_default_opts, A, lda, W, ldw, bias, M, K, x_inout, gamma, beta, eps, xn_bf16, st, prof);
+}
 int parseq_mlp_ln_bf16(const void* xn, const void* W1, const float* b1, const void* W2, const float* b2, int M, int D,
                        float* x_inout, const float* gamma, const float* beta, float eps, void* xn_out_bf16, parseq_stream_t stream) {
   PQ_TRY(ensure_kernel_attributes());
diff --git a/parseq_b200/csrc/gemm_ln.cuh b/parseq_b200/csrc/gemm_ln.cuh
--- a/parseq_b200/csrc/gemm_ln.cuh
+++ b/parseq_b200/csrc/gemm_ln.cuh
@@ -40,15 +40,15 @@
   static_assert(kStages >= 3, "pipeline depth");
 };
 
-template <int D>
-struct GemmLnCfg<D, 2> {
+template <int D, bool SHARED_W>
+struct GemmLnPairCfg {
   static_assert(D == 384, "the persistent column-split kernel is built for D = 384");
   static constexpr int kCG = 2;
-  static constexpr int kTileM = GLN_BLOCK_M;
+  static constexpr int kTileM = SHARED_W ? 2 * GLN_BLOCK_M : GLN_BLOCK_M;
   static constexpr int kCols = D / 2;
-  static constexpr int kABox = GLN_BLOCK_M;
+  static constexpr int kABox = kTileM;
   static constexpr int kBox = kCols;
-  static constexpr int kABytes = GLN_BLOCK_M * GEMM_BLOCK_K * 2;
+  static constexpr int kABytes = kTileM * GEMM_BLOCK_K * 2;
   static constexpr int kBBytes = kCols * GEMM_BLOCK_K * 2;
   static constexpr int kStageBytes = kABytes + kBBytes;
   static constexpr int kStages = 3;
@@ -60,8 +60,21 @@
   static constexpr int kSmemBytes = kStages * kStageBytes + 2 * kXBytes + kParamBytes + kBarBytes + 1024;
   static_assert(kSmemBytes <= 232448, "shared memory");
 };
+template <int D>
+struct GemmLnCfg<D, 2> : GemmLnPairCfg<D, false> {};
+template <int D>
+struct GemmLnCfg<D, 3> : GemmLnPairCfg<D, true> {};
+
+constexpr int GLN_SHARED_W_MIN_K = 768;
 
 constexpr int GLN_PARTS4_MIN_K = 768;
+
+constexpr int GLN_PROF_TILES = 32;
+__device__ __forceinline__ unsigned long long gln_timer_ns() {
+  unsigned long long t;
+  asm volatile("mov.u64 %0, %%globaltimer;" : "=l"(t));
+  return t;
+}
 
 template <int PARTS>
 __device__ __forceinline__ float gln_row_total(const float* s_part, int r) {
@@ -143,12 +156,12 @@
   }
 }
 
-template <int D, int PARTS>
+template <int D, int PARTS, bool PROF>
 __device__ __forceinline__ void gln_pair_epilogue(float (&acc)[D / 4], const uint8_t* xs, float* __restrict__ x,
                                                   __nv_bfloat16* __restrict__ xn, int M, float eps, int m0, int c0,
                                                   uint32_t rank, const float* s_bias, const float* s_gamma,
                                                   const float* s_beta, float* s_part, uint64_t* stat_bar, uint32_t par,
-                                                  uint64_t* x_empty) {
+                                                  uint64_t* x_empty, unsigned long long* ps) {
   using Cfg = GemmLnCfg<D, 2>;
   constexpr int kI = Cfg::kCols / 8;
   constexpr int kH = PARTS / 2;
@@ -161,6 +174,7 @@
   const uint8_t* xsa = xs + lr * 128 + (lane & 1) * 8;
   const uint8_t* xsb = xsa + 8 * 128;
   const uint32_t peer = rank ^ 1u;
+  constexpr uint32_t kPeerBytes = GLN_BLOCK_M * kH * 4;
 
   float sa[kH], sb[kH];
 #pragma unroll
@@ -183,6 +197,7 @@
     sb[h] += acc[4 * i + 2] + acc[4 * i + 3];
   }
   mbar_arrive(x_empty);
+  if constexpr (PROF) if (ps != nullptr && t == 0) ps[4] = gln_timer_ns();
   float mean_a = 0.f, mean_b = 0.f, rstd_a = 0.f, rstd_b = 0.f;
 #pragma unroll
   for (int round = 0; round < 2; ++round) {
@@ -199,6 +214,7 @@
       }
     }
     float* slots = s_part + round * PARTS * GLN_BLOCK_M;
+    const uint32_t peer_bar = mapa_cluster(smem_u32(&stat_bar[round]), peer);
 #pragma unroll
     for (int h = 0; h < kH; ++h) {
       sa[h] += __shfl_xor_sync(0xffffffffu, sa[h], 1);
@@ -209,13 +225,15 @@
       if ((lane & 3) == 0) {
         slot[lr] = sa[h];
         slot[lr + 8] = sb[h];
-        st_cluster_f32(mapa_cluster(smem_u32(slot + lr), peer), sa[h]);
-        st_cluster_f32(mapa_cluster(smem_u32(slot + lr + 8), peer), sb[h]);
-      }
-    }
-    mbar_arrive(&stat_bar[round]);
-    mbar_arrive_cluster(mapa_cluster(smem_u32(&stat_bar[round]), peer));
-    mbar_wait_cluster(&stat_bar[round], par);
+        const uint32_t peer_slot = mapa_cluster(smem_u32(slot + lr), peer);
+        st_async_cluster_f32(peer_slot, sa[h], peer_bar);
+        st_async_cluster_f32(peer_slot + 8 * sizeof(float), sb[h], peer_bar);
+      }
+    }
+    if (t == 0) mbar_expect_tx(&stat_bar[round], kPeerBytes);
+    else mbar_arrive(&stat_bar[round]);
+    mbar_wait_mma(&stat_bar[round], par);
+    if constexpr (PROF) if (ps != nullptr && t == 0) ps[5 + round] = gln_timer_ns();
     const float ta = gln_row_total<PARTS>(slots, lr), tb = gln_row_total<PARTS>(slots, lr + 8);
     if (round == 0) {
       mean_a = ta * (1.0f / D);
@@ -234,13 +252,15 @@
     if (ok_a) na[i * 4] = pack_bf16((acc[4 * i] - mean_a) * rstd_a * g0 + e0, (acc[4 * i + 1] - mean_a) * rstd_a * g1 + e1);
     if (ok_b) nb[i * 4] = pack_bf16((acc[4 * i + 2] - mean_b) * rstd_b * g0 + e0, (acc[4 * i + 3] - mean_b) * rstd_b * g1 + e1);
   }
-}
-
-template <int D>
+  if constexpr (PROF) if (ps != nullptr && t == 0) ps[7] = gln_timer_ns();
+}
+
+template <int D, int MODE, bool PROF>
 __device__ __forceinline__ void gln_pair_persistent(const CUtensorMap* tmA, const CUtensorMap* tmB, const CUtensorMap* tmX,
                                                     float* __restrict__ x, __nv_bfloat16* __restrict__ xn,
-                                                    const GemmLnParams& p) {
-  using Cfg = GemmLnCfg<D, 2>;
+                                                    const GemmLnParams& p, unsigned long long* prof) {
+  using Cfg = GemmLnCfg<D, MODE>;
+  constexpr bool kShared = MODE == 3;
   extern __shared__ uint8_t smem_raw[];
   const uint32_t raw_addr = smem_u32(smem_raw);
   const uint32_t pad = ((raw_addr + 1023u) & ~1023u) - raw_addr;
@@ -260,6 +280,9 @@
   const int cluster = static_cast<int>(blockIdx.x / Cfg::kCG), clusters = static_cast<int>(gridDim.x / Cfg::kCG);
   const int c0 = static_cast<int>(rank & 1u) * Cfg::kCols;
   const int num_kb = (p.K + GEMM_BLOCK_K - 1) / GEMM_BLOCK_K;
+  auto prof_row = [&](int j) -> unsigned long long* {
+    return (cluster == 0 && j < GLN_PROF_TILES) ? prof + (rank * GLN_PROF_TILES + j) * 16 : nullptr;
+  };
 
   grid_dep_launch();
   if (threadIdx.x == 0) {
@@ -268,13 +291,13 @@
     prefetch_tmap(tmX);
     for (int s = 0; s < Cfg::kStages; ++s) {
       mbar_init(&full_bar[s], 1);
-      mbar_init(&empty_bar[s], 1);
+      mbar_init(&empty_bar[s], kShared ? 2 : 1);
     }
     for (int w = 0; w < 2; ++w) {
       mbar_init(&x_full[w], 1);
       mbar_init(&x_empty[w], 128);
     }
-    for (int i = 0; i < 4; ++i) mbar_init(&stat_bar[i], 2 * 128);
+    for (int i = 0; i < 4; ++i) mbar_init(&stat_bar[i], 128);
     fence_mbar_init();
   }
   for (int j = threadIdx.x; j < Cfg::kCols; j += GLN_THREADS) {
@@ -293,19 +316,33 @@
       int j = 0;
       for (int tile = cluster; tile < p.num_m_tiles; tile += clusters, ++j) {
         const int m0 = tile * Cfg::kTileM;
-        const int w = j & 1;
-        mbar_wait_mma(&x_empty[w], ((j >> 1) & 1) ^ 1u);
-        mbar_expect_tx(&x_full[w], Cfg::kXBytes);
-#pragma unroll
-        for (int b = 0; b < Cfg::kCols / Cfg::kXBoxCols; ++b)
-          tma_load_2d(xs + w * Cfg::kXBytes + b * Cfg::kXBoxBytes, tmX, &x_full[w], c0 + b * Cfg::kXBoxCols, m0);
+        unsigned long long* ps = nullptr;
+        if constexpr (PROF) ps = prof_row(j);
+        auto load_x = [&](int w, uint32_t parity) {
+          mbar_wait_mma(&x_empty[w], parity);
+          if constexpr (PROF) if (ps != nullptr) ps[8] = gln_timer_ns();
+          mbar_expect_tx(&x_full[w], Cfg::kXBytes);
+#pragma unroll
+          for (int b = 0; b < Cfg::kCols / Cfg::kXBoxCols; ++b)
+            tma_load_2d(xs + w * Cfg::kXBytes + b * Cfg::kXBoxBytes, tmX, &x_full[w], c0 + b * Cfg::kXBoxCols,
+                        m0 + (kShared ? w * GLN_BLOCK_M : 0));
+        };
+        const int kb_x = kShared ? (num_kb < Cfg::kStages ? num_kb : Cfg::kStages) - 1 : -1;
+        if constexpr (!kShared) load_x(j & 1, ((j >> 1) & 1) ^ 1u);
         for (int kb = 0; kb < num_kb; ++kb) {
           mbar_wait_mma(&empty_bar[stage], phase ^ 1u);
           uint8_t* sa = smem + stage * Cfg::kStageBytes;
           mbar_expect_tx(&full_bar[stage], Cfg::kStageBytes);
           tma_load_2d(sa, tmA, &full_bar[stage], kb * GEMM_BLOCK_K, m0);
           tma_load_2d(sa + Cfg::kABytes, tmB, &full_bar[stage], kb * GEMM_BLOCK_K, c0);
+          if constexpr (PROF) if (ps != nullptr && (kb == 0 || kb == num_kb - 1)) ps[kb == 0 ? 9 : 10] = gln_timer_ns();
           if (++stage == Cfg::kStages) { stage = 0; phase ^= 1u; }
+          if constexpr (kShared) {
+            if (kb == kb_x) {
+              load_x(0, (j & 1) ^ 1u);
+              load_x(1, (j & 1) ^ 1u);
+            }
+          }
         }
       }
     }
@@ -318,20 +355,34 @@
     uint8_t* xw = xs + wg * Cfg::kXBytes;
     int stage = 0;
     uint32_t phase = 0, par = 0;
-    if (wg == 1) ring_advance(stage, phase, num_kb, Cfg::kStages);
+    if (!kShared && wg == 1) ring_advance(stage, phase, num_kb, Cfg::kStages);
+    const int tile_step = kShared ? clusters : 2 * clusters;
 #pragma unroll 1
-    for (int tile = cluster + wg * clusters; tile < p.num_m_tiles; tile += 2 * clusters) {
-      const int m0 = tile * Cfg::kTileM;
-      if (tile != cluster) named_bar_sync(1 + wg, 256);
+    for (int tile = cluster + (kShared ? 0 : wg * clusters); tile < p.num_m_tiles; tile += tile_step) {
+      const int m0 = tile * Cfg::kTileM + (kShared ? wg * GLN_BLOCK_M : 0);
+      unsigned long long* ps = nullptr;
+      unsigned long long waited = 0;
+      if constexpr (PROF) {
+        ps = (leader && (!kShared || wg == 0)) ? prof_row((tile - cluster) / clusters) : nullptr;
+        if (ps != nullptr) ps[12] = gln_timer_ns();
+      }
+      if (!kShared && tile != cluster) named_bar_sync(1 + wg, 256);
+      if constexpr (PROF) if (ps != nullptr) ps[0] = gln_timer_ns();
       float acc[Cfg::kCols / 2];
 #pragma unroll
       for (int i = 0; i < Cfg::kCols / 2; ++i) acc[i] = 0.0f;
       int prev = -1;
 #pragma unroll 1
       for (int kb = 0; kb < num_kb; ++kb) {
-        mbar_wait_mma(&full_bar[stage], phase);
+        if constexpr (PROF) {
+          const unsigned long long t0 = ps != nullptr ? gln_timer_ns() : 0ull;
+          mbar_wait_mma(&full_bar[stage], phase);
+          if (ps != nullptr) waited += gln_timer_ns() - t0;
+        } else {
+          mbar_wait_mma(&full_bar[stage], phase);
+        }
         const uint32_t base = smem_u32(smem + stage * Cfg::kStageBytes);
-        const uint64_t da = make_desc_k_sw128(base);
+        const uint64_t da = make_desc_k_sw128(base + (kShared ? wg * GLN_BLOCK_M * GEMM_BLOCK_K * 2 : 0));
         const uint64_t db = make_desc_k_sw128(base + Cfg::kABytes);
         wgmma_fence();
 #pragma unroll
@@ -346,18 +397,21 @@
         prev = stage;
         if (++stage == Cfg::kStages) { stage = 0; phase ^= 1u; }
       }
-      if (tile + clusters < p.num_m_tiles) named_bar_arrive(1 + (wg ^ 1), 256);
+      if constexpr (PROF) if (ps != nullptr) { ps[1] = gln_timer_ns(); ps[11] = waited; }
+      if (!kShared && tile + clusters < p.num_m_tiles) named_bar_arrive(1 + (wg ^ 1), 256);
       wgmma_wait<0>();
       wgmma_reg_fence(acc);
+      if constexpr (PROF) if (ps != nullptr) ps[2] = gln_timer_ns();
       if (leader) mbar_arrive(&empty_bar[prev]);
-      ring_advance(stage, phase, num_kb, Cfg::kStages);
+      if constexpr (!kShared) ring_advance(stage, phase, num_kb, Cfg::kStages);
       mbar_wait_mma(&x_full[wg], par);
+      if constexpr (PROF) if (ps != nullptr) ps[3] = gln_timer_ns();
       if (parts4)
-        gln_pair_epilogue<D, 4>(acc, xw, x, xn, p.M, p.eps, m0, c0, rank, s_bias, s_gamma, s_beta,
-                                s_part + wg * 2 * 4 * GLN_BLOCK_M, stat_bar + 2 * wg, par, &x_empty[wg]);
+        gln_pair_epilogue<D, 4, PROF>(acc, xw, x, xn, p.M, p.eps, m0, c0, rank, s_bias, s_gamma, s_beta,
+                                      s_part + wg * 2 * 4 * GLN_BLOCK_M, stat_bar + 2 * wg, par, &x_empty[wg], ps);
       else
-        gln_pair_epilogue<D, 2>(acc, xw, x, xn, p.M, p.eps, m0, c0, rank, s_bias, s_gamma, s_beta,
-                                s_part + wg * 2 * 4 * GLN_BLOCK_M, stat_bar + 2 * wg, par, &x_empty[wg]);
+        gln_pair_epilogue<D, 2, PROF>(acc, xw, x, xn, p.M, p.eps, m0, c0, rank, s_bias, s_gamma, s_beta,
+                                      s_part + wg * 2 * 4 * GLN_BLOCK_M, stat_bar + 2 * wg, par, &x_empty[wg], ps);
       par ^= 1u;
     }
   }
@@ -369,8 +423,9 @@
 gemm_ln_fused_kernel(const __grid_constant__ CUtensorMap tmA, const __grid_constant__ CUtensorMap tmB,
                      const __grid_constant__ CUtensorMap tmX, float* __restrict__ x, __nv_bfloat16* __restrict__ xn,
                      const GemmLnParams p) {
+  static_assert(MODE <= 2, "MODE 3 is gemm_ln_shared_w_kernel");
   if constexpr (MODE == 2) {
-    gln_pair_persistent<D>(&tmA, &tmB, &tmX, x, xn, p);
+    gln_pair_persistent<D, 2, false>(&tmA, &tmB, &tmX, x, xn, p, nullptr);
   } else {
     using Cfg = GemmLnCfg<D, MODE>;
     constexpr int kNW = Cfg::kNW;
@@ -446,4 +501,20 @@
   }
 }
 
-}
+template <int D>
+__global__ void __launch_bounds__(GLN_THREADS, 1)
+gemm_ln_shared_w_kernel(const __grid_constant__ CUtensorMap tmA, const __grid_constant__ CUtensorMap tmB,
+                        const __grid_constant__ CUtensorMap tmX, float* __restrict__ x, __nv_bfloat16* __restrict__ xn,
+                        const GemmLnParams p) {
+  gln_pair_persistent<D, 3, false>(&tmA, &tmB, &tmX, x, xn, p, nullptr);
+}
+
+template <int D, int MODE>
+__global__ void __launch_bounds__(GLN_THREADS, 1)
+gemm_ln_prof_kernel(const __grid_constant__ CUtensorMap tmA, const __grid_constant__ CUtensorMap tmB,
+                    const __grid_constant__ CUtensorMap tmX, float* __restrict__ x, __nv_bfloat16* __restrict__ xn,
+                    const GemmLnParams p, unsigned long long* prof) {
+  gln_pair_persistent<D, MODE, true>(&tmA, &tmB, &tmX, x, xn, p, prof);
+}
+
+}
diff --git a/parseq_b200/csrc/ptx.cuh b/parseq_b200/csrc/ptx.cuh
--- a/parseq_b200/csrc/ptx.cuh
+++ b/parseq_b200/csrc/ptx.cuh
@@ -207,24 +207,9 @@
       ::"r"(smem_u32(smem_dst)), "l"(reinterpret_cast<uint64_t>(tmap)), "r"(smem_u32(bar)), "r"(c0), "r"(c1), "h"(cta_mask)
       : "memory");
 }
-__device__ __forceinline__ void mbar_wait_cluster(uint64_t* bar, uint32_t parity) {
-  uint32_t ok = 0;
-  long long t0 = clock64();
-  uint32_t it = 0;
-  while (true) {
-    asm volatile(
-        "{\n\t.reg .pred p;\n\t"
-        "mbarrier.try_wait.parity.acquire.cluster.shared::cta.b64 p, [%1], %2;\n\t"
-        "selp.b32 %0, 1, 0, p;\n\t}"
-        : "=r"(ok)
-        : "r"(smem_u32(bar)), "r"(parity)
-        : "memory");
-    if (ok) return;
-    if (((++it) & 0x3ffu) == 0 && (clock64() - t0) > PQ_SPIN_LIMIT_CYCLES) __trap();
-  }
-}
-__device__ __forceinline__ void st_cluster_f32(uint32_t cluster_addr, float v) {
-  asm volatile("st.shared::cluster.f32 [%0], %1;" ::"r"(cluster_addr), "f"(v) : "memory");
+__device__ __forceinline__ void st_async_cluster_f32(uint32_t cluster_addr, float v, uint32_t cluster_bar) {
+  asm volatile("st.async.shared::cluster.mbarrier::complete_tx::bytes.b32 [%0], %1, [%2];"
+               ::"r"(cluster_addr), "r"(__float_as_uint(v)), "r"(cluster_bar) : "memory");
 }
 
 __device__ __forceinline__ uint64_t make_desc_k_sw128(uint32_t smem_addr) {
diff --git a/parseq_b200/engine.py b/parseq_b200/engine.py
--- a/parseq_b200/engine.py
+++ b/parseq_b200/engine.py
@@ -92,7 +92,7 @@
     "parseq_lexicon_check", "parseq_lexicon_create", "parseq_lexicon_destroy", "parseq_beam_search_lexicon",
     "parseq_beam_search_lexicon_u8",
     "parseq_postprocess", "parseq_encode", "parseq_decode", "parseq_decode_ex", "parseq_head", "parseq_text_embed", "parseq_kernel_launches", "parseq_debug_int", "parseq_bench_tma_stream",
-    "parseq_set_option", "parseq_get_timing", "parseq_get_ar_profile", "parseq_last_error", "parseq_version", "parseq_gemm_bf16", "parseq_gemm_ln_bf16", "parseq_mlp_ln_bf16", "parseq_layernorm_bf16",
+    "parseq_set_option", "parseq_get_timing", "parseq_get_ar_profile", "parseq_last_error", "parseq_version", "parseq_gemm_bf16", "parseq_gemm_ln_bf16", "parseq_gemm_ln_profile", "parseq_mlp_ln_bf16", "parseq_layernorm_bf16",
     "parseq_enc_attention", "parseq_qkv_attention_bf16", "parseq_head_lse_bf16", "parseq_head_topk_bf16",
     "parseq_beam_select",
 ]
@@ -163,6 +163,8 @@
                                      C.c_int64, C.c_void_p]
     lib.parseq_gemm_ln_bf16.argtypes = [C.c_void_p, C.c_int64, C.c_void_p, C.c_int64, C.c_void_p, C.c_int, C.c_int, C.c_int,
                                         C.c_void_p, C.c_void_p, C.c_void_p, C.c_float, C.c_void_p, C.c_void_p]
+    lib.parseq_gemm_ln_profile.argtypes = [C.c_void_p, C.c_int64, C.c_void_p, C.c_int64, C.c_void_p, C.c_int, C.c_int,
+                                           C.c_void_p, C.c_void_p, C.c_void_p, C.c_float, C.c_void_p, C.c_void_p, C.c_void_p]
     lib.parseq_mlp_ln_bf16.argtypes = [C.c_void_p, C.c_void_p, C.c_void_p, C.c_void_p, C.c_void_p, C.c_int, C.c_int, C.c_void_p,
                                        C.c_void_p, C.c_void_p, C.c_float, C.c_void_p, C.c_void_p]
     lib.parseq_layernorm_bf16.argtypes = [C.c_void_p, C.c_void_p, C.c_void_p, C.c_float, C.c_int, C.c_int,
```

Result: faster. 42110 (median of 6 runs) (+1.7%).
